# xUhEngwAng/I2V-Adapter-Unofficial

Measured on AMD Instinct MI355X. Metric: denoising steps/sec @ 16fx512x512 SD1.5+I2V-Adapter, higher is better.
Workload: dtype f16

## Files before the change

i2v-adapter-unofficial_amd/_lib.py:

```python
import ctypes as C
import os

_HERE = os.path.dirname(os.path.abspath(__file__))
LIB_PATH = os.environ.get("I2V_LIB_PATH") or os.path.join(_HERE, "libi2v_hip.so")
ABI_VERSION = 11

I2V_EPI_NONE, I2V_EPI_GELU, I2V_EPI_GEGLU = 0, 1, 2
I2V_STORE_ROWMAJOR, I2V_STORE_ROWPERM, I2V_STORE_VT, I2V_STORE_VT_T = 0, 1, 2, 3
I2V_A_PLAIN, I2V_A_CONV3X3 = 0, 1


class HipLibraryError(RuntimeError):
    pass


class GemmParams(C.Structure):
    _fields_ = [
        ("a", C.c_void_p), ("lda", C.c_int64),
        ("a2", C.c_void_p), ("lda2", C.c_int64),
        ("k_split", C.c_int32), ("a_mode", C.c_int32),
        ("w", C.c_void_p), ("ldw", C.c_int64),
        ("bias", C.c_void_p),
        ("residual", C.c_void_p), ("ldr", C.c_int64),
        ("rowvec", C.c_void_p), ("ld_rowvec", C.c_int64), ("rows_per_vec", C.c_int32), ("rowvec_period", C.c_int32),
        ("ln_wsum", C.c_void_p), ("ln_eps", C.c_float),
        ("c", C.c_void_p), ("ldc", C.c_int64),
        ("M", C.c_int32), ("N", C.c_int32), ("K", C.c_int32),
        ("epilogue", C.c_int32), ("store_mode", C.c_int32),
        ("frames", C.c_int32), ("hw", C.c_int32),
        ("vt_len", C.c_int32), ("vt_ld", C.c_int32),
        ("out_scale", C.c_float),
        ("n_img", C.c_int32), ("in_h", C.c_int32), ("in_w", C.c_int32), ("cin", C.c_int32),
        ("out_h", C.c_int32), ("out_w", C.c_int32), ("stride", C.c_int32), ("upsample", C.c_int32),
        ("asym_pad", C.c_int32), ("conv_kblock", C.c_int32),
        ("w_batch_stride", C.c_int64), ("rows_per_w", C.c_int32),
        ("a_perm_frames", C.c_int32), ("a_perm_hw", C.c_int32),
        ("workspace", C.c_void_p), ("workspace_bytes", C.c_int64),
        ("c_is_f32", C.c_int32),
        ("gn_partial", C.c_void_p), ("gn_groups", C.c_int32),
        ("residual_lo", C.c_void_p), ("c_lo", C.c_void_p),
    ]


class AttnParams(C.Structure):
    _fields_ = [
        ("q", C.c_void_p), ("q_row_stride", C.c_int64), ("q_batch_stride", C.c_int64),
        ("k", C.c_void_p), ("k_row_stride", C.c_int64), ("k_batch_stride", C.c_int64),
        ("vt", C.c_void_p), ("vt_row_stride", C.c_int64), ("vt_batch_stride", C.c_int64),
        ("o", C.c_void_p), ("o_row_stride", C.c_int64), ("o_batch_stride", C.c_int64),
        ("batch_q", C.c_int32), ("kv_group", C.c_int32), ("heads", C.c_int32), ("head_dim", C.c_int32),
        ("lq", C.c_int32), ("lk", C.c_int32),
        ("scale", C.c_float), ("accumulate", C.c_int32), ("acc_scale", C.c_float),
        ("lse", C.c_void_p),
    ]


class AttnBwdParams(C.Structure):
    _fields_ = [
        ("q", C.c_void_p), ("q_row_stride", C.c_int64), ("q_batch_stride", C.c_int64),
        ("qt", C.c_void_p), ("qt_row_stride", C.c_int64), ("qt_batch_stride", C.c_int64),
        ("k", C.c_void_p), ("k_row_stride", C.c_int64), ("k_batch_stride", C.c_int64),
        ("kt", C.c_void_p), ("kt_row_stride", C.c_int64), ("kt_batch_stride", C.c_int64),
        ("v", C.c_void_p), ("v_row_stride", C.c_int64), ("v_batch_stride", C.c_int64),
        ("dout", C.c_void_p), ("do_row_stride", C.c_int64), ("do_batch_stride", C.c_int64),
        ("doutt", C.c_void_p), ("dot_row_stride", C.c_int64), ("dot_batch_stride", C.c_int64),
        ("lse", C.c_void_p), ("delta", C.c_void_p),
        ("dq", C.c_void_p), ("dq_row_stride", C.c_int64), ("dq_batch_stride", C.c_int64),
        ("dk", C.c_void_p), ("dk_row_stride", C.c_int64), ("dk_batch_stride", C.c_int64),
        ("dv", C.c_void_p), ("dv_row_stride", C.c_int64), ("dv_batch_stride", C.c_int64),
        ("batch_q", C.c_int32), ("kv_group", C.c_int32), ("heads", C.c_int32), ("head_dim", C.c_int32),
        ("lq", C.c_int32), ("lk", C.c_int32),
        ("scale", C.c_float), ("kv_partitions", C.c_int32), ("dkv_partial", C.c_void_p),
    ]


class TAttnParams(C.Structure):
    _fields_ = [
        ("q", C.c_void_p), ("q_row_stride", C.c_int64),
        ("k", C.c_void_p), ("k_row_stride", C.c_int64),
        ("vt", C.c_void_p), ("vt_ld", C.c_int32),
        ("o", C.c_void_p), ("o_row_stride", C.c_int64),
        ("n_pixels", C.c_int32), ("frames", C.c_int32), ("heads", C.c_int32), ("head_dim", C.c_int32),
        ("scale", C.c_float),
    ]


class MotionAttnParams(C.Structure):
    _fields_ = [
        ("x", C.c_void_p), ("ldx", C.c_int64),
        ("gamma", C.c_void_p),
        ("shift", C.c_void_p), ("ld_shift", C.c_int64),
        ("w_qkv", C.c_void_p),
        ("out", C.c_void_p), ("ldo", C.c_int64),
        ("rows", C.c_int64),
        ("channels", C.c_int32), ("heads", C.c_int32), ("head_dim", C.c_int32), ("frames", C.c_int32),
        ("eps", C.c_float), ("scale", C.c_float),
        ("w_o", C.c_void_p), ("b_o", C.c_void_p),
    ]


class CrossAttnFusedParams(C.Structure):
    _fields_ = [
        ("x", C.c_void_p), ("ldx", C.c_int64),
        ("gamma", C.c_void_p), ("beta", C.c_void_p),
        ("w_q", C.c_void_p),
        ("ctx_frag", C.c_void_p),
        ("out", C.c_void_p), ("ldo", C.c_int64),
        ("rows", C.c_int64), ("rows_per_ctx", C.c_int64),
        ("channels", C.c_int32), ("heads", C.c_int32), ("head_dim", C.c_int32), ("ctx_len", C.c_int32),
        ("eps", C.c_float), ("scale", C.c_float),
        ("ip_frag", C.c_void_p), ("ip_len", C.c_int32), ("ip_scale", C.c_float),
        ("w_o", C.c_void_p), ("b_o", C.c_void_p),
    ]


class FfFusedParams(C.Structure):
    _fields_ = [
        ("x", C.c_void_p), ("ldx", C.c_int64),
        ("gamma", C.c_void_p), ("beta", C.c_void_p),
        ("w1", C.c_void_p), ("b1", C.c_void_p),
        ("w2", C.c_void_p), ("b2", C.c_void_p),
        ("out", C.c_void_p), ("ldo", C.c_int64),
        ("rows", C.c_int64),
        ("channels", C.c_int32), ("inner", C.c_int32),
        ("eps", C.c_float),
        ("w3", C.c_void_p), ("b3", C.c_void_p),
        ("res2", C.c_void_p), ("ld_res2", C.c_int64),
        ("perm_frames", C.c_int32), ("perm_hw", C.c_int32),
        ("res2_lo", C.c_void_p), ("out_lo", C.c_void_p),
    ]


class LnQkvParams(C.Structure):
    _fields_ = [
        ("x", C.c_void_p), ("ldx", C.c_int64),
        ("gamma", C.c_void_p), ("beta", C.c_void_p),
        ("w", C.c_void_p),
        ("qk", C.c_void_p), ("ld_qk", C.c_int64),
        ("vt", C.c_void_p), ("vt_batch_stride", C.c_int64), ("vt_row_stride", C.c_int64),
        ("rows", C.c_int64), ("rows_per_image", C.c_int64),
        ("channels", C.c_int32), ("n_qk", C.c_int32),
        ("eps", C.c_float),
        ("x_image_stride", C.c_int64),
    ]


class UnetConfig(C.Structure):
    _fields_ = [
        ("in_channels", C.c_int32), ("out_channels", C.c_int32),
        ("block_out_channels", C.c_int32 * 4),
        ("layers_per_block", C.c_int32), ("num_attention_heads", C.c_int32),
        ("cross_attention_dim", C.c_int32), ("norm_num_groups", C.c_int32),
        ("motion_max_seq_length", C.c_int32), ("motion_num_attention_heads", C.c_int32),
        ("use_motion_mid_block", C.c_int32), ("ip_num_tokens", C.c_int32),
    ]


class UnetPlan(C.Structure):
    _fields_ = [
        ("batch", C.c_int32), ("frames", C.c_int32), ("height", C.c_int32), ("width", C.c_int32),
        ("ctx_len", C.c_int32), ("has_ip", C.c_int32),
    ]


class GnParams(C.Structure):
    _fields_ = [
        ("x", C.c_void_p), ("c1", C.c_int32),
        ("x2", C.c_void_p), ("c2", C.c_int32),
        ("gamma", C.c_void_p), ("beta", C.c_void_p),
        ("y", C.c_void_p),
        ("n_img", C.c_int32), ("hw", C.c_int32), ("groups", C.c_int32), ("frames_per_stat", C.c_int32),
        ("eps", C.c_float), ("silu", C.c_int32),
        ("out_perm", C.c_int32), ("frames", C.c_int32),
        ("workspace", C.c_void_p),
        ("gpartial_in", C.c_void_p), ("gpartial_rows", C.c_int32),
    ]


class LnParams(C.Structure):
    _fields_ = [
        ("x", C.c_void_p), ("ldx", C.c_int64),
        ("gamma", C.c_void_p), ("beta", C.c_void_p),
        ("pe", C.c_void_p), ("ld_pe", C.c_int64), ("pe_period", C.c_int32),
        ("y", C.c_void_p), ("ldy", C.c_int64),
        ("rows", C.c_int32), ("C", C.c_int32),
        ("eps", C.c_float),
        ("x_rows_per_batch", C.c_int32), ("x_batch_stride", C.c_int64),
    ]


_P = C.c_void_p
SIGNATURES = {
    "i2v_abi_version": (C.c_int, []),
    "i2v_last_error": (C.c_char_p, []),
    "i2v_gemm_f16": (C.c_int, [C.POINTER(GemmParams), _P]),
    "i2v_gemm_ln_supported": (C.c_int, [C.POINTER(GemmParams)]),
    "i2v_gemm_batch_supported": (C.c_int, [C.POINTER(GemmParams)]),
    "i2v_gemm_upconv_fold_supported": (C.c_int, [C.POINTER(GemmParams)]),
    "i2v_gemm_workspace_bytes": (C.c_int64, [C.POINTER(GemmParams)]),
    "i2v_gemm_gn_partial_rows": (C.c_int32, [C.POINTER(GemmParams)]),
    "i2v_attention_f16": (C.c_int, [C.POINTER(AttnParams), _P]),
    "i2v_temporal_attention_f16": (C.c_int, [C.POINTER(TAttnParams), _P]),
    "i2v_motion_attn_supported": (C.c_int32, [C.c_int64, C.c_int32, C.c_int32, C.c_int32, C.c_int32]),
    "i2v_motion_attn_pack_rows": (C.c_int32, [C.c_int32, C.c_int32]),
    "i2v_motion_attn_f16": (C.c_int, [C.POINTER(MotionAttnParams), _P]),
    "i2v_cross_attn_fused_supported": (C.c_int32, [C.c_int64, C.c_int32, C.c_int32, C.c_int32, C.c_int32, C.c_int64]),
    "i2v_cross_attn_fused_pack_rows": (C.c_int32, [C.c_int32, C.c_int32]),
    "i2v_cross_attn_fused_ctx_elems": (C.c_int64, [C.c_int32, C.c_int32, C.c_int32]),
    "i2v_cross_attn_fused_f16": (C.c_int, [C.POINTER(CrossAttnFusedParams), _P]),
    "i2v_ln_qkv_supported": (C.c_int32, [C.c_int64, C.c_int32, C.c_int32, C.c_int64]),
    "i2v_ln_qkv_f16": (C.c_int, [C.POINTER(LnQkvParams), _P]),
    "i2v_ff_fused_supported": (C.c_int32, [C.c_int64, C.c_int32, C.c_int32]),
    "i2v_ff_fused_tail_supported": (C.c_int32, [C.c_int64, C.c_int32, C.c_int32, C.c_int32, C.c_int32]),
    "i2v_ff_fused_f16": (C.c_int, [C.POINTER(FfFusedParams), _P]),
    "i2v_groupnorm_workspace_bytes": (C.c_int64, [C.c_int32, C.c_int32, C.c_int32]),
    "i2v_groupnorm_f16": (C.c_int, [C.POINTER(GnParams), _P]),
    "i2v_groupnorm_fold_f16": (C.c_int, [C.POINTER(GnParams), _P, C.c_int64, _P, C.c_int32, _P, _P, _P]),
    "i2v_layernorm_f16": (C.c_int, [C.POINTER(LnParams), _P]),
    "i2v_softmax_rows_f16": (C.c_int, [_P, C.c_int64, _P, C.c_int64, C.c_int32, C.c_int32, C.c_float, _P]),
    "i2v_nchw_to_tokens": (C.c_int, [_P, C.c_int32, _P, C.c_int32, C.c_int32, C.c_int32, C.c_int32, _P]),
    "i2v_tokens_to_nchw": (C.c_int, [_P, C.c_int32, C.c_int64, _P, C.c_int32, C.c_int32, C.c_int32, C.c_int32, _P]),
    "i2v_timestep_embedding": (C.c_int, [_P, _P, C.c_int32, _P, C.c_int32, C.c_int32, _P]),
    "i2v_silu_f16": (C.c_int, [_P, _P, C.c_int64, _P]),
    "i2v_repeat_rows_f16": (C.c_int, [_P, _P, C.c_int64, C.c_int64, C.c_int32, _P]),
    "i2v_copy3d_f16": (C.c_int, [_P, C.c_int64, C.c_int64, _P, C.c_int64, C.c_int64, C.c_int64, C.c_int64,
                                 C.c_int64, _P]),
    "i2v_pack_ctx_fragments_elems": (C.c_int64, [C.c_int32, C.c_int32, C.c_int32]),
    "i2v_pack_ctx_fragments_f16": (C.c_int, [_P, C.c_int64, _P, C.c_int64, C.c_int64, _P, C.c_int32, C.c_int32, C.c_int32, C.c_int32, _P]),
    "i2v_ddim_prep": (C.c_int, [_P, _P, _P, C.c_int32, C.c_int32, C.c_int32, C.c_int32, C.c_int32, C.c_int32, _P]),
    "i2v_gaussian_sample_f32": (C.c_int, [_P, _P, _P, C.c_int32, C.c_int32, C.c_int32, _P]),
    "i2v_first_frame_prior_f32": (C.c_int, [_P, _P, _P, _P, C.c_int32, C.c_int32, C.c_int32, C.c_int32, C.c_int32,
                                            C.c_float, C.c_float, C.c_float, C.c_float, C.c_float, _P]),
    "i2v_attention_lse_f32": (C.c_int, [C.POINTER(AttnParams), _P, _P]),
    "i2v_attention_bwd_f16": (C.c_int, [C.POINTER(AttnBwdParams), _P]),
    "i2v_transpose_f16": (C.c_int, [_P, C.c_int64, C.c_int64, _P, C.c_int64, C.c_int64, C.c_int32, C.c_int32, C.c_int32, _P]),
    "i2v_rowdot_heads_f32": (C.c_int, [_P, C.c_int64, _P, C.c_int64, _P, C.c_int64, C.c_int32, C.c_int32, C.c_int32, _P]),
    "i2v_layernorm_bwd_f16": (C.c_int, [_P, C.c_int64, _P, C.c_int64, _P, _P, C.c_int64, _P, C.c_int64, C.c_int32, C.c_int32,
                                        C.c_float, _P]),
    "i2v_geglu_bwd_f16": (C.c_int, [_P, C.c_int64, _P, C.c_int64, _P, C.c_int64, C.c_int64, C.c_int32, _P]),
    "i2v_geglu_f16": (C.c_int, [_P, C.c_int64, _P, C.c_int64, C.c_int64, C.c_int32, _P]),
    "i2v_colsum_f32": (C.c_int, [_P, C.c_int64, _P, C.c_int64, C.c_int32, _P]),
    "i2v_colsum_prod_f32": (C.c_int, [_P, C.c_int64, _P, C.c_int64, _P, C.c_int64, C.c_int32, _P]),
    "i2v_colsum_workspace_bytes": (C.c_int64, [C.c_int64, C.c_int32]),
    "i2v_colsum_det_f32": (C.c_int, [_P, C.c_int64, _P, C.c_int64, _P, C.c_int64, C.c_int32, _P, _P]),
    "i2v_masked_mse_grad_f16": (C.c_int, [_P, _P, _P, C.c_int64, C.c_int32, C.c_int32, C.c_int32, C.c_float, _P]),
    "i2v_masked_mse_grad_f32": (C.c_int, [_P, _P, _P, _P, C.c_int64, C.c_int32, C.c_int32, C.c_int32, C.c_float, _P]),
    "i2v_groupnorm_bwd_workspace_bytes": (C.c_int64, [C.c_int32, C.c_int32, C.c_int32]),
    "i2v_groupnorm_bwd_f16": (C.c_int, [C.POINTER(GnParams), _P, _P, _P, _P]),
    "i2v_add_f16": (C.c_int, [_P, _P, _P, C.c_int64, _P]),
    "i2v_permute_rows_f16": (C.c_int, [_P, _P, C.c_int64, C.c_int32, C.c_int32, C.c_int32, C.c_int32, _P]),
    "i2v_zero_insert2x_f16": (C.c_int, [_P, _P, C.c_int64, C.c_int32, C.c_int32, C.c_int32, _P]),
    "i2v_sum_pool2x_f16": (C.c_int, [_P, _P, C.c_int64, C.c_int32, C.c_int32, C.c_int32, _P]),
    "i2v_sumsq_f32": (C.c_int, [_P, C.c_int64, _P, _P]),
    "i2v_adamw_f32": (C.c_int, [_P, _P, _P, _P, C.c_int64, C.c_float, C.c_float, C.c_float, C.c_float, C.c_float, C.c_int32,
                                C.c_float, _P, C.c_float, _P]),
    "i2v_adamw_guarded_f32": (C.c_int, [_P, _P, _P, _P, C.c_int64, C.c_float, C.c_float, C.c_float, C.c_float, C.c_float,
                                        C.c_float, C.c_float, _P, C.c_int32, _P, _P, _P, _P]),
    "i2v_axpby_f32": (C.c_int, [_P, _P, C.c_float, C.c_float, C.c_int64, _P]),
    "i2v_select_row_f16": (C.c_int, [_P, C.c_int64, C.c_int32, _P, _P, C.c_int32, _P]),
    "i2v_ddim_cfg_step": (C.c_int, [_P, _P, C.c_int32, C.c_int64, _P, C.c_int32, _P, C.c_float, C.c_int32, C.c_int32,
                                    C.c_int32, C.c_int32, C.c_int32, _P]),
    "i2v_dpm_cfg_step": (C.c_int, [_P, _P, _P, C.c_int32, C.c_int64, _P, C.c_int32, _P, C.c_float, C.c_int32, C.c_int32,
                                   C.c_int32, C.c_int32, C.c_int32, _P]),
    "i2v_freeu_f16": (C.c_int, [_P, _P, _P, _P, _P, _P, C.c_int32, C.c_int32, C.c_int32, C.c_int32, C.c_int32, C.c_float, C.c_float, _P]),
    "i2v_unet_create": (C.c_int, [C.POINTER(UnetConfig), C.POINTER(_P)]),
    "i2v_unet_destroy": (C.c_int, [_P]),
    "i2v_unet_set_weight": (C.c_int, [_P, C.c_char_p, _P, C.c_int32, C.c_int32, C.POINTER(C.c_int64)]),
    "i2v_unet_get_weight": (C.c_int, [_P, C.c_char_p, C.POINTER(_P), C.POINTER(C.c_int32), C.POINTER(C.c_int32),
                                      C.POINTER(C.c_int64)]),
    "i2v_unet_num_weights": (C.c_int64, [_P]),
    "i2v_unet_plan": (C.c_int, [_P, C.POINTER(UnetPlan)]),
    "i2v_unet_set_plan": (C.c_int, [_P, C.c_char_p, C.c_int64]),
    "i2v_unet_activation_bytes": (C.c_int64, [_P]),
    "i2v_unet_plan_launches": (C.c_int32, [_P]),
    "i2v_unet_plan_num_keys": (C.c_int32, [_P]),
    "i2v_unet_plan_key": (C.c_char_p, [_P, C.c_int32]),
    "i2v_unet_set_workspace": (C.c_int, [_P, _P, C.c_int64]),
    "i2v_unet_forward": (C.c_int, [_P, _P, _P, _P, _P, _P, _P]),
    "i2v_unet_abort_capture": (C.c_int, [_P]),
    "i2v_unet_run": (C.c_int, [_P, C.POINTER(_P), C.c_int32, _P]),
    "i2v_unet_capture_step": (C.c_int, [_P, _P]),
    "i2v_unet_end_capture": (C.c_int, [_P]),
    "i2v_unet_replay_step": (C.c_int, [_P, _P]),
    "i2v_unet_has_step": (C.c_int32, [_P]),
}

_lib = None


def load():
    global _lib
    if _lib is not None:
        return _lib
    if not os.path.exists(LIB_PATH):
        raise HipLibraryError(
            f"{LIB_PATH} not found: the HIP extension is not built.  Run `python __graft_entry__.py build` "
            "(needs hipcc, cross-compiles gfx950 without a GPU).  There is no CPU fallback for this path.")
    try:
        lib = C.CDLL(LIB_PATH)
    except OSError as e:
        raise HipLibraryError(f"cannot load {LIB_PATH}: {e}") from e
    for name, (res, args) in SIGNATURES.items():
        try:
            fn = getattr(lib, name)
        except AttributeError as e:
            raise HipLibraryError(f"{LIB_PATH} does not export `{name}` declared in include/i2v_hip.h") from e
        fn.restype = res
        fn.argtypes = args
    v = lib.i2v_abi_version()
    if v != ABI_VERSION:
        raise HipLibraryError(f"{LIB_PATH} has ABI version {v}, binding expects {ABI_VERSION}")
    _lib = lib
    return lib


def check(status: int, what: str):
    if status != 0:
        msg = load().i2v_last_error()
        raise HipLibraryError(f"{what} failed with status {status}: {msg.decode() if msg else ''}")
```

i2v-adapter-unofficial_amd/blocks.py:

```python
import math
import os
from typing import Optional

import torch
from torch import nn

from . import kernels as K
from . import streams
from ._lib import (I2V_EPI_GEGLU, I2V_EPI_GELU, I2V_EPI_NONE, I2V_STORE_ROWPERM, HipLibraryError)
from .checkpoint import PretrainedMixin

f16 = torch.float16


class HipModule(nn.Module):

    def __init__(self):
        super().__init__()
        self._packed = None
        self._packed_key = None

    def _pack(self):
        return {}

    def __getstate__(self):
        state = self.__dict__.copy()
        state["_packed"], state["_packed_key"] = None, None
        return state

    def packed(self):
        key = tuple((p.data_ptr(), p._version, p.dtype) for p in self.parameters())
        key += tuple((b.data_ptr(), b._version) for b in self.buffers())
        if self._packed is None or key != self._packed_key:
            for p in self.parameters():
                if not p.is_cuda:
                    raise HipLibraryError(
                        f"{type(self).__name__} has parameters on {p.device}: the HIP path has no CPU fallback")
            with torch.no_grad():
                self._packed = self._pack()
            self._packed_key = key
        return self._packed


def w16(t: torch.Tensor) -> torch.Tensor:
    return t.detach().to(f16).contiguous()


class LazyPack(dict):

    def __init__(self, *a, **kw):
        super().__init__(*a, **kw)
        self._lazy = {}

    def lazy(self, name, fn):
        self._lazy[name] = (fn, None)

    def lazy_group(self, names, fn):
        for i, n in enumerate(names):
            self._lazy[n] = (fn, (tuple(names), i))

    def __missing__(self, key):
        if key not in self._lazy:
            raise KeyError(key)
        fn, grp = self._lazy[key]
        with torch.no_grad():
            val = fn()
        if grp is None:
            del self._lazy[key]
            self[key] = val
        else:
            for n, v in zip(grp[0], val):
                self._lazy.pop(n, None)
                dict.__setitem__(self, n, v)
        return dict.__getitem__(self, key)

    def __contains__(self, key):
        return dict.__contains__(self, key) or key in self._lazy

    def get(self, key, default=None):
        return self[key] if key in self else default


def pack_conv3x3(weight: torch.Tensor, cin_pad: Optional[int] = None) -> torch.Tensor:
    co, ci = weight.shape[:2]
    w = weight.detach().permute(0, 2, 3, 1)
    if cin_pad is not None and cin_pad != ci:
        w = torch.nn.functional.pad(w, (0, cin_pad - ci))
        ci = cin_pad
    if K.conv_k_block(ci):
        w = w.reshape(co, 9, ci // 64, 64).permute(0, 2, 1, 3)
    return w.reshape(co, 9 * ci).to(f16).contiguous()


def pack_upconv_fold(weight: torch.Tensor, dtype=f16) -> torch.Tensor:
    co, ci = weight.shape[:2]
    w = weight.detach()
    w = w.double() if w.dtype == torch.float64 else w.float()
    rows = (((0,), (1, 2)), ((0, 1), (2,)))
    phases = []
    for py in range(2):
        for px in range(2):
            taps = []
            for ty in range(2):
                for tx in range(2):
                    acc = None
                    for ky in rows[py][ty]:
                        for kx in rows[px][tx]:
                            acc = w[:, :, ky, kx] if acc is None else acc + w[:, :, ky, kx]
                    taps.append(acc)
            phases.append(torch.stack(taps, dim=1))
    f = torch.stack(phases, dim=0)
    if K.conv_k_block(ci):
        f = f.reshape(4, co, 4, ci // 64, 64).permute(0, 1, 3, 2, 4)
    return f.reshape(4, co, 4 * ci).to(dtype).contiguous()


UPCONV_FOLD = os.environ.get("I2V_UPCONV_FOLD", "1") != "0"


def pack_geglu(weight, bias):
    inner = weight.shape[0] // 2
    w = torch.stack([weight[:inner], weight[inner:]], dim=1).reshape(2 * inner, weight.shape[1])
    b = torch.stack([bias[:inner], bias[inner:]], dim=1).reshape(2 * inner)
    return w16(w), w16(b)


LN_FOLD = os.environ.get("I2V_LN_FOLD", "1") != "0"


def fold_layernorm(weight, bias, gamma, beta):
    wf = (weight.detach().float() * gamma.detach().float()[None, :]).to(f16).contiguous()
    wsum = wf.float().sum(dim=1).contiguous()
    b = weight.detach().float() @ beta.detach().float()
    if bias is not None:
        b = b + bias.detach().float()
    return wf, wsum, b.to(f16).contiguous()


def fold_layernorm_geglu(proj_weight, proj_bias, gamma, beta):
    wf, wsum, b = fold_layernorm(proj_weight, proj_bias, gamma, beta)
    inner = wf.shape[0] // 2
    il = lambda t: torch.stack([t[:inner], t[inner:]], dim=1).reshape((2 * inner,) + tuple(t.shape[1:])).contiguous()
    return il(wf), il(wsum), il(b)


class LnFoldPlan:

    def __init__(self):
        self._cache = {}

    def get(self, key, probe):
        if not LN_FOLD:
            return False
        if key not in self._cache:
            self._cache[key] = bool(probe())
        return self._cache[key]


class ProjectedContext:

    def __init__(self, text, ip):
        self.text, self.ip = text, ip
        self.kv = {}
        self.frag = {}

    @property
    def shape(self):
        return self.text.shape


class ProjectedTemb:

    def __init__(self, all_proj, slices):
        self.all_proj, self.slices = all_proj, slices

    def view_for(self, resnet):
        off, n = self.slices[resnet]
        return self.all_proj[:, off: off + n]

    def first_half(self):
        r = self.all_proj.shape[0]
        return self if r == 1 else ProjectedTemb(self.all_proj[: r // 2], self.slices)


GN_FOLD = os.environ.get("I2V_GN_FOLD", "1") != "0"
GN_FOLD_RATIO = float(os.environ.get("I2V_GN_FOLD_RATIO", "4"))


def gn_proj_in(x, gamma, beta, groups, eps, w, bias, frames=0):
    n, hh, ww, c = x.shape
    hw = hh * ww
    fps = frames if frames > 0 else 1
    s_groups, n_out = n // fps, w.shape[0]
    if GN_FOLD and GN_FOLD_RATIO * s_groups * n_out <= n * hw:
        kw = dict(rows_per_vec=fps * hw, w_rows=fps * hw, a_perm=(frames, hw) if frames > 0 else None)
        if _fold_supported(x, s_groups, n_out, kw):
            w_s, b_s = K.groupnorm_fold(x, gamma, beta, groups, eps, w, bias, frames_per_stat=fps)
            return K.gemm(x.view(-1, c), w_s, None, rowvec=b_s, **kw)
    if frames > 0:
        h = K.groupnorm(x, gamma, beta, groups, eps, frames_per_stat=frames, out_perm=True, frames=frames)
    else:
        h = K.groupnorm(x, gamma, beta, groups, eps).view(-1, c)
    return K.gemm(h, w, bias)


_FOLD_OK = {}


def _fold_supported(x, s_groups, n_out, kw):
    key = (tuple(x.shape), s_groups, n_out, kw["w_rows"], kw["a_perm"])
    ok = _FOLD_OK.get(key)
    if ok is None:
        c = x.shape[3]
        w_s = torch.empty((s_groups, n_out, c), dtype=f16, device=x.device)
        b_s = torch.empty((s_groups, n_out), dtype=f16, device=x.device)
        ok = _FOLD_OK[key] = K.gemm(x.view(-1, c), w_s, None, rowvec=b_s, query_batch_support=True, **kw)
    return ok


def to_tokens(x: torch.Tensor, c_pad: Optional[int] = None) -> torch.Tensor:
    return K.nchw_to_tokens(x, c_pad)


def from_tokens(x: torch.Tensor, dtype) -> torch.Tensor:
    return K.tokens_to_nchw(x, dtype=dtype if dtype in (torch.float32, f16) else f16)


def _as_f16_matrix(t: torch.Tensor) -> torch.Tensor:
    if not t.is_cuda:
        raise HipLibraryError(f"tensor on {t.device}: the HIP path has no CPU fallback")
    return t.to(f16).contiguous()


class Timesteps(nn.Module):

    def __init__(self, num_channels: int, flip_sin_to_cos: bool = True, downscale_freq_shift: float = 0):
        super().__init__()
        if not flip_sin_to_cos or downscale_freq_shift != 0:
            raise NotImplementedError("hot path uses Timesteps(C, flip_sin_to_cos=True, freq_shift=0)")
        self.num_channels = num_channels

    def forward(self, timesteps: torch.Tensor) -> torch.Tensor:
        return K.timestep_embedding(timesteps.to(torch.float32).contiguous(), self.num_channels)


class TimestepEmbedding(HipModule):

    def __init__(self, in_channels: int, time_embed_dim: int, act_fn: str = "silu"):
        super().__init__()
        self.linear_1 = nn.Linear(in_channels, time_embed_dim)
        self.act = nn.SiLU()
        self.linear_2 = nn.Linear(time_embed_dim, time_embed_dim)

    def _pack(self):
        return dict(w1=w16(self.linear_1.weight), b1=w16(self.linear_1.bias), w2=w16(self.linear_2.weight),
                    b2=w16(self.linear_2.bias))

    def forward(self, sample, condition=None):
        p = self.packed()
        h = K.silu(K.gemm(_as_f16_matrix(sample), p["w1"], p["b1"]))
        return K.gemm(h, p["w2"], p["b2"])


_PRECISE_STREAM = os.environ.get("I2V_STREAM_PRECISE", "0") != "0"


def precise_stream() -> bool:
    return _PRECISE_STREAM


def set_precise_stream(on: bool) -> bool:
    global _PRECISE_STREAM
    prev, _PRECISE_STREAM = _PRECISE_STREAM, bool(on)
    return prev


GN_FROM_CONV = os.environ.get("I2V_GN_FROM_CONV", "1") != "0"


class ResnetBlock2D(HipModule):

    def __init__(self, in_channels, out_channels=None, temb_channels=512, eps=1e-6, groups=32,
                 output_scale_factor=1.0, **_unused):
        super().__init__()
        out_channels = in_channels if out_channels is None else out_channels
        self.in_channels, self.out_channels = in_channels, out_channels
        self.output_scale_factor = output_scale_factor
        self.groups, self.eps = groups, eps
        self.norm1 = nn.GroupNorm(groups, in_channels, eps=eps, affine=True)
        self.conv1 = nn.Conv2d(in_channels, out_channels, 3, stride=1, padding=1)
        self.time_emb_proj = nn.Linear(temb_channels, out_channels) if temb_channels is not None else None
        self.norm2 = nn.GroupNorm(groups, out_channels, eps=eps, affine=True)
        self.conv2 = nn.Conv2d(out_channels, out_channels, 3, stride=1, padding=1)
        self.nonlinearity = nn.SiLU()
        self.conv_shortcut = (nn.Conv2d(in_channels, out_channels, 1, stride=1, padding=0)
                              if in_channels != out_channels else None)

    def _pack(self):
        p = dict(g1=w16(self.norm1.weight), b1=w16(self.norm1.bias), w1=pack_conv3x3(self.conv1.weight),
                 cb1=w16(self.conv1.bias), g2=w16(self.norm2.weight), b2=w16(self.norm2.bias),
                 w2=pack_conv3x3(self.conv2.weight), cb2=w16(self.conv2.bias))
        if self.time_emb_proj is not None:
            p["wt"], p["bt"] = w16(self.time_emb_proj.weight), w16(self.time_emb_proj.bias)
        if self.conv_shortcut is not None:
            p["ws"] = w16(self.conv_shortcut.weight.reshape(self.out_channels, self.in_channels))
            p["bs"] = w16(self.conv_shortcut.bias)
        return p

    def _fwd(self, x, temb_act, x2=None):
        p = self.packed()
        n, hh, ww, c1 = x.shape
        cin = c1 + (x2.shape[3] if x2 is not None else 0)
        if cin != self.in_channels:
            raise ValueError(f"ResnetBlock2D expects {self.in_channels} input channels, got {cin}")
        if self.conv_shortcut is None and x2 is not None:
            raise ValueError("concat input needs a conv_shortcut")
        s = x
        with streams.fork(self.conv_shortcut is not None and n * hh * ww <= streams.MAX_ROWS, x.device) as fk:
            if self.conv_shortcut is not None:
                with fk.side():
                    a2 = None if x2 is None else x2.view(-1, x2.shape[3])
                    s = K.sview(K.gemm(x.view(-1, c1), p["ws"], p["bs"], a2=a2, precise=precise_stream()), n, hh, ww, self.out_channels)
            h = K.groupnorm(x, p["g1"], p["b1"], self.groups, self.eps, x2=x2, silu=True)
            rowvec, rpv = None, 0
            if self.time_emb_proj is not None and temb_act is not None:
                rowvec = (temb_act.view_for(self) if isinstance(temb_act, ProjectedTemb)
                          else K.gemm(temb_act, p["wt"], p["bt"]))
                rpv = (n // rowvec.shape[0]) * hh * ww
            if GN_FROM_CONV:
                h, st = K.conv3x3(h, p["w1"], p["cb1"], rowvec=rowvec, rows_per_vec=rpv, gn_stats_groups=self.groups)
            else:
                h, st = K.conv3x3(h, p["w1"], p["cb1"], rowvec=rowvec, rows_per_vec=rpv), None
            h = K.groupnorm(h, p["g2"], p["b2"], self.groups, self.eps, silu=True, stats=st)
        return K.conv3x3(h, p["w2"], p["cb2"], residual=s, out_scale=1.0 / self.output_scale_factor, precise=precise_stream())

    def forward(self, input_tensor, temb, scale: float = 1.0):
        x = to_tokens(input_tensor)
        ta = K.silu(_as_f16_matrix(temb)) if temb is not None else None
        return from_tokens(self._fwd(x, ta), input_tensor.dtype)


class Downsample2D(HipModule):

    def __init__(self, channels, use_conv=True, out_channels=None, padding=1, name="conv"):
        super().__init__()
        if not use_conv or padding not in (0, 1):
            raise NotImplementedError("Downsample2D(use_conv=True, padding in {0, 1}) only")
        out_channels = out_channels or channels
        self.padding = padding
        self.conv = nn.Conv2d(channels, out_channels, 3, stride=2, padding=padding)

    def _pack(self):
        return dict(w=pack_conv3x3(self.conv.weight), b=w16(self.conv.bias))

    def _fwd(self, x):
        p = self.packed()
        return K.conv3x3(x, p["w"], p["b"], stride=2, asym_pad=self.padding == 0, precise=precise_stream())

    def forward(self, hidden_states, scale: float = 1.0):
        return from_tokens(self._fwd(to_tokens(hidden_states)), hidden_states.dtype)


class Upsample2D(HipModule):

    def __init__(self, channels, use_conv=True, out_channels=None):
        super().__init__()
        if not use_conv:
            raise NotImplementedError("hot path uses Upsample2D(use_conv=True)")
        out_channels = out_channels or channels
        self.conv = nn.Conv2d(channels, out_channels, 3, padding=1)

    def _pack(self):
        p = LazyPack(w=pack_conv3x3(self.conv.weight), b=w16(self.conv.bias))
        p.lazy("w_fold", lambda: pack_upconv_fold(self.conv.weight))
        return p

    def _fwd(self, x, output_size=None):
        p = self.packed()
        size = None if output_size is None else tuple(int(v) for v in output_size)
        if (UPCONV_FOLD and size in (None, (2 * x.shape[1], 2 * x.shape[2]))
                and K.upconv_fold_supported(x.shape, self.conv.out_channels)):
            return K.conv3x3(x, p["w"], p["b"], upsample=True, w_folded=p["w_fold"])
        return K.conv3x3(x, p["w"], p["b"], upsample=True, output_size=size)

    def forward(self, hidden_states, output_size=None, scale: float = 1.0):
        return from_tokens(self._fwd(to_tokens(hidden_states), output_size), hidden_states.dtype)


class Attention(HipModule):

    def __init__(self, query_dim, cross_attention_dim=None, heads=8, dim_head=64, bias=False, out_bias=True,
                 dropout=0.0, upcast_attention=False):
        super().__init__()
        if bias:
            raise NotImplementedError("attention_bias=True is not on the hot path")
        self.inner_dim = dim_head * heads
        self.heads, self.dim_head = heads, dim_head
        self.query_dim = query_dim
        self.cross_attention_dim = cross_attention_dim if cross_attention_dim is not None else query_dim
        self.scale = dim_head ** -0.5
        self.to_q = nn.Linear(query_dim, self.inner_dim, bias=False)
        self.to_k = nn.Linear(self.cross_attention_dim, self.inner_dim, bias=False)
        self.to_v = nn.Linear(self.cross_attention_dim, self.inner_dim, bias=False)
        self.to_out = nn.ModuleList([nn.Linear(self.inner_dim, query_dim, bias=out_bias), nn.Dropout(dropout)])
        self.ip_num_tokens, self.ip_scale = 0, 1.0
        self.to_k_ip = None
        self.to_v_ip = None

    def install_ip_adapter(self, to_k_ip_weight, to_v_ip_weight, num_tokens=4, scale=1.0):
        dev, dt = self.to_q.weight.device, self.to_q.weight.dtype
        self.to_k_ip = nn.Linear(self.cross_attention_dim, self.inner_dim, bias=False).to(device=dev, dtype=dt)
        self.to_v_ip = nn.Linear(self.cross_attention_dim, self.inner_dim, bias=False).to(device=dev, dtype=dt)
        with torch.no_grad():
            self.to_k_ip.weight.copy_(to_k_ip_weight)
            self.to_v_ip.weight.copy_(to_v_ip_weight)
        self.ip_num_tokens, self.ip_scale = num_tokens, scale

    def _pack(self):
        ob = self.to_out[0].bias
        p = dict(wq=w16(self.to_q.weight), wk=w16(self.to_k.weight), wv=w16(self.to_v.weight),
                 wo=w16(self.to_out[0].weight), bo=None if ob is None else w16(ob))
        if self.to_k_ip is not None:
            p["wk_ip"], p["wv_ip"] = w16(self.to_k_ip.weight), w16(self.to_v_ip.weight)
        return p

    def project_kv(self, ctx_text, ctx_ip, out=None):
        p = self.packed()
        bc, lt, dc = ctx_text.shape
        o = out if out is not None else (None, None, None, None)
        k = K.gemm(ctx_text.view(-1, dc), p["wk"], out=o[0])
        vt = K.project_vt(ctx_text.view(-1, dc), p["wv"], lt, out=o[1])
        kip = vtip = None
        if ctx_ip is not None and self.ip_num_tokens:
            kip = K.gemm(ctx_ip.view(-1, dc), p["wk_ip"], out=o[2])
            vtip = K.project_vt(ctx_ip.view(-1, dc), p["wv_ip"], ctx_ip.shape[1], out=o[3])
        return k, vt, kip, vtip

    def context_kv(self, ctx_text, ctx_ip):
        if isinstance(ctx_text, ProjectedContext):
            k, vt, kip, vtip = ctx_text.kv[self]
            lt = ctx_text.text.shape[1]
            li = ctx_text.ip.shape[1] if ctx_text.ip is not None else 0
        else:
            k, vt, kip, vtip = self.project_kv(ctx_text, ctx_ip)
            lt = ctx_text.shape[1]
            li = ctx_ip.shape[1] if ctx_ip is not None else 0
        return k, vt, kip, vtip, lt, li

    def context_fragments(self, ctx_text, kv):
        k, vt, kip, vtip, lt, li = kv
        use_ip = kip is not None and bool(self.ip_num_tokens)
        if not isinstance(ctx_text, ProjectedContext):
            return K.pack_ctx_fragments(k, vt, self.heads, lt), (K.pack_ctx_fragments(kip, vtip, self.heads, li) if use_ip else None)
        hit = ctx_text.frag.get(self)
        if hit is None:
            hit = ctx_text.frag[self] = (K.pack_ctx_fragments(k, vt, self.heads, lt),
                                         K.pack_ctx_fragments(kip, vtip, self.heads, li) if use_ip else None)
        return hit

    def refresh_context_fragments(self, pc):
        hit = pc.frag.get(self)
        if hit is not None:
            k, vt, kip, vtip, lt, li = self.context_kv(pc, None)
            K.pack_ctx_fragments(k, vt, self.heads, lt, out=hit[0])
            if hit[1] is not None:
                K.pack_ctx_fragments(kip, vtip, self.heads, li, out=hit[1])

    def _cross(self, q, ctx_text, ctx_ip, batch_q, lq, kv_group, kv=None):
        k, vt, kip, vtip, lt, li = kv if kv is not None else self.context_kv(ctx_text, ctx_ip)
        o = K.attention(q, k, vt, batch_q=batch_q, lq=lq, lk=lt, heads=self.heads, head_dim=self.dim_head,
                        kv_group=kv_group, scale=self.scale)
        if kip is not None and self.ip_num_tokens:
            K.attention(q, kip, vtip, batch_q=batch_q, lq=lq, lk=li, heads=self.heads, head_dim=self.dim_head,
                        kv_group=kv_group, scale=self.scale, out=o, accumulate=True, acc_scale=self.ip_scale)
        return o

    def forward(self, hidden_states, encoder_hidden_states=None, attention_mask=None):
        if attention_mask is not None:
            raise NotImplementedError("attention masks are never passed on the hot path (SURVEY 8b)")
        p = self.packed()
        x = _as_f16_matrix(hidden_states)
        b, l, c = x.shape
        q = K.gemm(x.view(-1, c), p["wq"])
        ctx = x if encoder_hidden_states is None else _as_f16_matrix(encoder_hidden_states)
        ctx_ip = None
        if self.ip_num_tokens and encoder_hidden_states is not None:
# ... 656 lines not shown
```

i2v-adapter-unofficial_amd/csrc/gemm.hip:

```cpp
#include <cstdlib>

#include "gemm_common.h"

namespace {

constexpr int BK = 64;

template <int BM, int BN>
struct Smem {
  f16 a[2][BM * BK];
  f16 w[2][BN * BK];
};

__device__ __forceinline__ int swz(int row, int chunk) { return row * 128 + ((chunk ^ ((row >> 1) & 7)) << 4); }

struct ConvRow {
  int pix_base;
  int oy, ox;
  bool valid;
};

template <int BM, int BN, int AMODE>
__global__ __launch_bounds__(256) void gemm_kernel(const i2v_gemm_params p, const int tiles_n, const int vec4) {
  constexpr int WM = BM / 2, WN = BN / 2, MI = WM / 16, NI = WN / 16;
// ... 185 lines not shown
          for (int r = 0; r < 4; ++r) v[r] += (float)b4[r];
        }
        if (rv) {
          const f16x4 t4 = *reinterpret_cast<const f16x4*>(rv + n);
#pragma unroll
          for (int r = 0; r < 4; ++r) v[r] += (float)t4[r];
        }
        if (rs) {
          const f16x4 r4 = *reinterpret_cast<const f16x4*>(rs + n);
#pragma unroll
          for (int r = 0; r < 4; ++r) v[r] += (float)r4[r];
          if (rl) {
            const f16x4 l4 = *reinterpret_cast<const f16x4*>(rl + n);
#pragma unroll
            for (int r = 0; r < 4; ++r) v[r] += (float)l4[r];
          }
        }
      } else {
#pragma unroll
        for (int r = 0; r < 4; ++r) {
          if (n + r < N) {
            if (bias) v[r] += (float)bias[n + r];
            if (rv) v[r] += (float)rv[n + r];
            if (rs) v[r] += (float)rs[n + r];
            if (rl) v[r] += (float)rl[n + r];
          }
        }
      }
      if (p.epilogue == I2V_EPI_GEGLU) {
        const float o0 = v[0] * gelu_erf(v[1]) * oscale;
        const float o1 = v[2] * gelu_erf(v[3]) * oscale;
        f16* dst = C + m_out * p.ldc + (n >> 1);
        if (vec4) {
          f16x2 o = {(f16)o0, (f16)o1};
          *reinterpret_cast<f16x2*>(dst) = o;
        } else {
          if (n + 1 < N) dst[0] = (f16)o0;
          if (n + 3 < N) dst[1] = (f16)o1;
        }
        continue;
      }
#pragma unroll
      for (int r = 0; r < 4; ++r) {
        if (p.epilogue == I2V_EPI_GELU) v[r] = gelu_erf(v[r]);
        v[r] *= oscale;
      }
      if (p.store_mode == I2V_STORE_VT_T) {
        const int bt = m / p.vt_len, kk = m - bt * p.vt_len;
#pragma unroll
        for (int r = 0; r < 4; ++r)
          if (n + r < N) C[((int64_t)bt * N + (n + r)) * p.vt_ld + kk] = (f16)v[r];
      } else if (p.store_mode == I2V_STORE_VT) {
        if (vec4) {
          const int bt = n / p.vt_len, kk = n - bt * p.vt_len;
          f16x4 o = {(f16)v[0], (f16)v[1], (f16)v[2], (f16)v[3]};
          *reinterpret_cast<f16x4*>(C + ((int64_t)bt * M + m) * p.vt_ld + kk) = o;
        } else {
#pragma unroll
          for (int r = 0; r < 4; ++r) {
            if (n + r < N) {
              const int bt = (n + r) / p.vt_len, kk = (n + r) - bt * p.vt_len;
              C[((int64_t)bt * M + m) * p.vt_ld + kk] = (f16)v[r];
            }
          }
        }
      } else if (p.c_is_f32) {
        float* dst = reinterpret_cast<float*>(p.c) + m_out * p.ldc + n;
        if (vec4) {
          *reinterpret_cast<f32x4*>(dst) = f32x4{v[0], v[1], v[2], v[3]};
        } else {
#pragma unroll
          for (int r = 0; r < 4; ++r)
            if (n + r < N) dst[r] = v[r];
        }
      } else {
        f16* dst = C + m_out * p.ldc + n;
        if (vec4) {
          f16x4 o = {(f16)v[0], (f16)v[1], (f16)v[2], (f16)v[3]};
          *reinterpret_cast<f16x4*>(dst) = o;
          if (cl) *reinterpret_cast<f16x4*>(cl + n) = f16x4{lo_half(v[0], o[0]), lo_half(v[1], o[1]), lo_half(v[2], o[2]), lo_half(v[3], o[3])};
        } else {
#pragma unroll
          for (int r = 0; r < 4; ++r)
            if (n + r < N) {
              dst[r] = (f16)v[r];
              if (cl) cl[n + r] = lo_half(v[r], (f16)v[r]);
            }
        }
      }
    }
  }
}

struct TileCfg {
  int bm, bn, blocks_per_cu;
  float eff;
};

template <int BM, int BN>
int launch(const i2v_gemm_params& p, int vec4, hipStream_t s) {
  const int tiles_m = (int)i2v_cdiv(p.M, BM), tiles_n = (int)i2v_cdiv(p.N, BN);
  const dim3 grid(tiles_m * tiles_n), block(256);
  if (p.a_mode == I2V_A_CONV3X3)
    hipLaunchKernelGGL((gemm_kernel<BM, BN, I2V_A_CONV3X3>), grid, block, 0, s, p, tiles_n, vec4);
  else
    hipLaunchKernelGGL((gemm_kernel<BM, BN, I2V_A_PLAIN>), grid, block, 0, s, p, tiles_n, vec4);
  return i2v_check_launch("i2v_gemm_f16");
}

inline bool aligned_to(const void* p, uintptr_t a) { return (reinterpret_cast<uintptr_t>(p) % a) == 0; }

int vector_epilogue_ok(const i2v_gemm_params& p) {
  int vec4 = (p.N % 4 == 0) ? 1 : 0;
  if (p.bias && !aligned_to(p.bias, 8)) vec4 = 0;
  if (p.residual && (!aligned_to(p.residual, 8) || p.ldr % 4 != 0)) vec4 = 0;
  if ((p.residual_lo && !aligned_to(p.residual_lo, 8)) || (p.c_lo && !aligned_to(p.c_lo, 8))) vec4 = 0;
  if (p.rowvec && (!aligned_to(p.rowvec, 8) || p.ld_rowvec % 4 != 0)) vec4 = 0;
  if (p.store_mode == I2V_STORE_VT) {
    if (p.vt_len % 4 != 0 || p.vt_ld % 4 != 0 || !aligned_to(p.c, 8)) vec4 = 0;
  } else if (p.store_mode == I2V_STORE_VT_T) {
    vec4 = (p.vt_len % 4 == 0 && p.vt_ld % 4 == 0 && aligned_to(p.c, 8) && p.M % 4 == 0) ? 1 : 0;
  } else if (p.epilogue == I2V_EPI_GEGLU) {
    if (p.ldc % 2 != 0 || !aligned_to(p.c, 4)) vec4 = 0;
  } else if (p.c_is_f32) {
    if (p.ldc % 4 != 0 || !aligned_to(p.c, 16)) vec4 = 0;
  } else {
    if (p.ldc % 4 != 0 || !aligned_to(p.c, 8)) vec4 = 0;
  }
  return vec4;
}

}

extern "C" int64_t i2v_gemm_workspace_bytes(const i2v_gemm_params* pp) {
  if (pp == nullptr || pp->M <= 0 || pp->N <= 0 || pp->K <= 0) return 0;
  return i2v_gemm_big_plan(*pp, vector_epilogue_ok(*pp)).workspace_bytes;
}

extern "C" int i2v_gemm_ln_supported(const i2v_gemm_params* pp) {
  if (pp == nullptr || pp->M <= 0 || pp->N <= 0 || pp->K <= 0) return 0;
  return i2v_gemm_big_plan(*pp, vector_epilogue_ok(*pp)).ln_fold ? 1 : 0;
}

extern "C" int i2v_gemm_batch_supported(const i2v_gemm_params* pp) {
  if (pp == nullptr || pp->M <= 0 || pp->N <= 0 || pp->K <= 0) return 0;
  return i2v_gemm_big_plan(*pp, vector_epilogue_ok(*pp)).form == GemmBigForm::Tile ? 1 : 0;
}

extern "C" int i2v_gemm_upconv_fold_supported(const i2v_gemm_params* pp) {
  if (pp == nullptr || pp->M <= 0 || pp->N <= 0 || pp->K <= 0 || pp->a_mode != I2V_A_CONV3X3 || pp->upsample != 2) return 0;
  return i2v_gemm_big_plan(*pp, vector_epilogue_ok(*pp)).form == GemmBigForm::Tile ? 1 : 0;
}

extern "C" int32_t i2v_gemm_gn_partial_rows(const i2v_gemm_params* pp) {
  if (pp == nullptr) return 0;
  return i2v_gemm_big_plan(*pp, vector_epilogue_ok(*pp)).gn_rows;
}

extern "C" int i2v_gemm_f16(const i2v_gemm_params* pp, i2v_stream_t stream) {
  I2V_CHECK_ARG(pp != nullptr, "i2v_gemm_f16: null params");
  const i2v_gemm_params& p = *pp;
  I2V_CHECK_ARG(p.a && p.w && p.c, "i2v_gemm_f16: null a/w/c pointer");
  I2V_CHECK_ARG(p.M > 0 && p.N > 0 && p.K > 0, "i2v_gemm_f16: M, N, K must be positive (got %d, %d, %d)", p.M, p.N,
                p.K);
  I2V_CHECK_ARG(p.K % 8 == 0, "i2v_gemm_f16: K (%d) must be a multiple of 8", p.K);
  I2V_CHECK_ARG(p.ldw % 8 == 0 && p.ldw >= p.K, "i2v_gemm_f16: ldw (%lld) must be >= K and a multiple of 8",
                (long long)p.ldw);
  I2V_CHECK_ARG(aligned_to(p.a, 16) && aligned_to(p.w, 16), "i2v_gemm_f16: a / w must be 16-byte aligned");
  I2V_CHECK_ARG(p.lda % 8 == 0, "i2v_gemm_f16: lda (%lld) must be a multiple of 8", (long long)p.lda);
  if (p.a_mode == I2V_A_CONV3X3) {
    I2V_CHECK_ARG(p.a2 == nullptr, "i2v_gemm_f16: conv mode takes a single source");
    I2V_CHECK_ARG(p.upsample >= 0 && p.upsample <= 2, "i2v_gemm_f16: upsample must be 0, 1 or 2 (got %d)", p.upsample);
    I2V_CHECK_ARG(p.cin > 0 && p.cin % 8 == 0 && p.K == (p.upsample == 2 ? 4 : 9) * p.cin,
                  "i2v_gemm_f16: conv needs cin %% 8 == 0, K == 9 cin (4 cin with the up-sampling folded into the weights)");
    I2V_CHECK_ARG(p.stride == 1 || p.stride == 2, "i2v_gemm_f16: conv stride must be 1 or 2");
    I2V_CHECK_ARG(!(p.upsample && p.stride != 1), "i2v_gemm_f16: upsample conv must have stride 1");
    I2V_CHECK_ARG(!p.asym_pad || (p.stride == 2 && !p.upsample), "i2v_gemm_f16: asym_pad needs stride 2, no upsample");
    I2V_CHECK_ARG(p.conv_kblock == 0 || (p.conv_kblock == 64 && p.cin % 64 == 0),
                  "i2v_gemm_f16: conv_kblock must be 0 or 64 (with cin %% 64 == 0), got %d for cin %d", p.conv_kblock, p.cin);
    const int padsum = p.asym_pad ? 1 : 2;
    const int eh = p.upsample ? 2 * p.in_h : (p.in_h + padsum - 3) / p.stride + 1;
    const int ew = p.upsample ? 2 * p.in_w : (p.in_w + padsum - 3) / p.stride + 1;
    I2V_CHECK_ARG((p.out_h == eh || (p.upsample == 1 && p.out_h == eh - 1)) && (p.out_w == ew || (p.upsample == 1 && p.out_w == ew - 1)),
                  "i2v_gemm_f16: conv output size mismatch (%d x %d vs %d x %d)", p.out_h, p.out_w, eh, ew);
    I2V_CHECK_ARG((int64_t)p.n_img * p.out_h * p.out_w == p.M, "i2v_gemm_f16: conv M != n_img*out_h*out_w");
    I2V_CHECK_ARG(p.lda >= p.cin, "i2v_gemm_f16: conv pixel stride lda < cin");
    I2V_CHECK_ARG((int64_t)p.n_img * p.in_h * p.in_w < (1ll << 31), "i2v_gemm_f16: conv image too large");
  } else {
    I2V_CHECK_ARG(p.a_mode == I2V_A_PLAIN, "i2v_gemm_f16: bad a_mode %d", p.a_mode);
    if (p.a2) {
      I2V_CHECK_ARG(p.k_split > 0 && p.k_split < p.K && p.k_split % 8 == 0 && p.lda2 % 8 == 0 && aligned_to(p.a2, 16),
                    "i2v_gemm_f16: bad dual-source split (k_split %d, K %d)", p.k_split, p.K);
      I2V_CHECK_ARG(p.lda >= p.k_split && p.lda2 >= p.K - p.k_split, "i2v_gemm_f16: dual-source ld too small");
    } else {
      I2V_CHECK_ARG(p.lda >= p.K, "i2v_gemm_f16: lda (%lld) < K (%d)", (long long)p.lda, p.K);
    }
  }
  I2V_CHECK_ARG(p.epilogue >= I2V_EPI_NONE && p.epilogue <= I2V_EPI_GEGLU, "i2v_gemm_f16: bad epilogue");
  I2V_CHECK_ARG(p.store_mode >= I2V_STORE_ROWMAJOR && p.store_mode <= I2V_STORE_VT_T, "i2v_gemm_f16: bad store_mode");
  if (p.epilogue == I2V_EPI_GEGLU)
    I2V_CHECK_ARG(p.N % 2 == 0 && p.store_mode != I2V_STORE_VT && p.store_mode != I2V_STORE_VT_T,
                  "i2v_gemm_f16: GEGLU needs even N, non-VT store");
  if (p.store_mode == I2V_STORE_VT_T) {
    I2V_CHECK_ARG(p.vt_len > 0 && p.vt_ld >= p.vt_len && p.M % p.vt_len == 0,
                  "i2v_gemm_f16: VT_T store needs M %% vt_len == 0 and vt_ld >= vt_len");
    I2V_CHECK_ARG(p.residual == nullptr && (p.rowvec == nullptr || (p.rowvec_period > 0 && p.ln_wsum)),
                  "i2v_gemm_f16: VT_T store takes no residual, and a rowvec only as the transposed positional table of a "
                  "LayerNorm-folded projection");
  }
  if (p.c_is_f32)
    I2V_CHECK_ARG(p.c_is_f32 == 1 && p.epilogue != I2V_EPI_GEGLU && p.store_mode == I2V_STORE_ROWMAJOR && p.ln_wsum == nullptr &&
                      p.rows_per_w == 0 && p.a_perm_frames == 0 && p.N <= 64 && aligned_to(p.c, 4),
                  "i2v_gemm_f16: an fp32 result (c_is_f32) is a row-major store of a narrow (N <= 64), plain problem");
  if (p.residual_lo || p.c_lo) {
    I2V_CHECK_ARG(p.residual_lo == nullptr || p.residual != nullptr, "i2v_gemm_f16: residual_lo needs residual");
    I2V_CHECK_ARG(p.epilogue == I2V_EPI_NONE && (p.store_mode == I2V_STORE_ROWMAJOR || p.store_mode == I2V_STORE_ROWPERM) && !p.c_is_f32 &&
                      p.ln_wsum == nullptr && p.gn_partial == nullptr,
                  "i2v_gemm_f16: the precise residual stream (residual_lo / c_lo) takes plain row-major / row-permuted fp16 stores only");
  }
  if (p.rowvec) I2V_CHECK_ARG(p.rows_per_vec > 0 || p.rowvec_period > 0, "i2v_gemm_f16: rows_per_vec must be positive");
  if (p.store_mode == I2V_STORE_ROWPERM) {
    I2V_CHECK_ARG(p.frames > 0 && p.hw > 0 && p.M % (p.frames * p.hw) == 0,
                  "i2v_gemm_f16: ROWPERM needs M %% (frames*hw) == 0");
    I2V_CHECK_ARG(p.rowvec == nullptr, "i2v_gemm_f16: ROWPERM does not take rowvec");
  }
  if (p.store_mode == I2V_STORE_VT) {
    I2V_CHECK_ARG(p.vt_len > 0 && p.vt_ld >= p.vt_len && p.N % p.vt_len == 0,
                  "i2v_gemm_f16: VT store needs N %% vt_len == 0 and vt_ld >= vt_len");
    I2V_CHECK_ARG(p.residual == nullptr && p.rowvec == nullptr, "i2v_gemm_f16: VT store takes no residual/rowvec");
  }

  int vec4 = vector_epilogue_ok(p);
  const GemmBigPlan big_plan = i2v_gemm_big_plan(p, vec4);
  if (p.rowvec && p.rowvec_period > 0)
    I2V_CHECK_ARG(p.store_mode != I2V_STORE_ROWPERM && p.store_mode != I2V_STORE_VT &&
                      (p.rowvec_period & (p.rowvec_period - 1)) == 0,
                  "i2v_gemm_f16: a periodic rowvec (positional table) needs a power-of-two period (the epilogue masks the "
                  "row index: an integer modulo there cost the 256-row kernels 40 %%) and a row-major / VT_T store");
  if (p.ln_wsum) {
    I2V_CHECK_ARG(aligned_to(p.ln_wsum, 16) && p.ln_eps > 0.f, "i2v_gemm_f16: ln_wsum must be 16-byte aligned, ln_eps > 0");
    if (!big_plan.ln_fold)
      I2V_FAIL(I2V_ERR_INVALID_ARG, "i2v_gemm_f16: LayerNorm-folded GEMM is not implemented for this problem "
               "(M %d N %d K %d, epilogue %d, store %d): ask i2v_gemm_ln_supported() first", p.M, p.N, p.K, p.epilogue,
               p.store_mode);
  }

  if (p.gn_partial) {
    I2V_CHECK_ARG(aligned_to(p.gn_partial, 8), "i2v_gemm_f16: gn_partial must be 8-byte aligned");
    if (!big_plan.gn_rows)
      I2V_FAIL(I2V_ERR_INVALID_ARG, "i2v_gemm_f16: GroupNorm partials (gn_partial) are not implemented for this problem (M %d N %d K %d, "
               "groups %d): ask i2v_gemm_gn_partial_rows() first", p.M, p.N, p.K, p.gn_groups);
  }
  if (p.a_mode == I2V_A_CONV3X3 && p.upsample == 2 && big_plan.form != GemmBigForm::Tile)
    I2V_FAIL(I2V_ERR_INVALID_ARG, "i2v_gemm_f16: the folded up-sampling convolution (upsample = 2) is not implemented for this problem "
             "(M %d N %d cin %d, %d x %d -> %d x %d, rows_per_w %d): ask i2v_gemm_upconv_fold_supported() first", p.M, p.N, p.cin,
             p.in_h, p.in_w, p.out_h, p.out_w, p.rows_per_w);
  if (p.rows_per_w > 0 || p.a_perm_frames > 0) {
    I2V_CHECK_ARG(p.rows_per_w >= 0 && p.a_perm_frames >= 0 && p.w_batch_stride >= 0, "i2v_gemm_f16: negative batch / permutation field");
    if (big_plan.form != GemmBigForm::Tile)
      I2V_FAIL(I2V_ERR_INVALID_ARG, "i2v_gemm_f16: per-batch weights / the permuted A gather are not implemented for this "
               "problem (M %d N %d K %d, rows_per_w %d, a_perm %d x %d): they need the 8-wave kernel with full row tiles",
               p.M, p.N, p.K, p.rows_per_w, p.a_perm_frames, p.a_perm_hw);
  }
#ifdef I2V_VARIANTS
  {
    const int ws = i2v_gemm_ws_try(p, reinterpret_cast<hipStream_t>(stream));
    if (ws != 0) return ws < 0 ? ws : I2V_OK;
  }
#endif
  {
    const int thin = i2v_conv_thin_try(p, reinterpret_cast<hipStream_t>(stream));
    if (thin != 0) return thin < 0 ? thin : I2V_OK;
  }
  {
    const int big = i2v_gemm_big_launch(p, vec4, big_plan, reinterpret_cast<hipStream_t>(stream));
    if (big != 0) return big < 0 ? big : I2V_OK;
  }
  if (p.store_mode == I2V_STORE_VT_T) vec4 = 0;
  const bool conv = p.a_mode == I2V_A_CONV3X3;
  const bool long_k = p.K >= 2048;
  const TileCfg cfgs[4] = {{128, 128, 2, long_k ? 1.15f : 1.00f},
                           {128, 64, 3, conv ? 1.00f : 1.30f},
                           {64, 128, 3, conv ? 1.25f : 1.25f},
                           {64, 64, 5, 1.10f}};
  int best = 0;
  double best_t = 1e300;
  for (int i = 0; i < 4; ++i) {
    const double tiles = (double)i2v_cdiv(p.M, cfgs[i].bm) * (double)i2v_cdiv(p.N, cfgs[i].bn);
    const double slots = 256.0 * cfgs[i].blocks_per_cu;
    const double rounds = tiles <= slots ? 1.0 : tiles / slots;
    const double conc = tiles < slots ? tiles : slots;
    const double per_cu = (conc / 256.0 < 1.0) ? 1.0 : conc / 256.0;
    const double t = rounds * per_cu * cfgs[i].bm * cfgs[i].bn / cfgs[i].eff;
    if (t < best_t) {
      best_t = t;
      best = i;
    }
  }
  static const int tile_env = getenv("I2V_GEMM_TILE") ? atoi(getenv("I2V_GEMM_TILE")) : -1;
  if (tile_env >= 0 && tile_env < 4) best = tile_env;
  hipStream_t s = reinterpret_cast<hipStream_t>(stream);
  switch (best) {
    case 0: return launch<128, 128>(p, vec4, s);
    case 1: return launch<128, 64>(p, vec4, s);
    case 2: return launch<64, 128>(p, vec4, s);
    default: return launch<64, 64>(p, vec4, s);
  }
}
```

i2v-adapter-unofficial_amd/csrc/gemm_big.hip:

```cpp
#include <algorithm>
#include <cstdlib>
#include <utility>

#include "gemm_common.h"

namespace {

constexpr int BIG_BN = 320;

__device__ __forceinline__ void bdma16(__amdgpu_buffer_rsrc_t rsrc, char* lds_wave_base, unsigned voff, int soff) {
  __builtin_amdgcn_raw_ptr_buffer_load_lds(rsrc, (__attribute__((address_space(3))) void*)lds_wave_base, 16, voff, soff, 0,
                                           0);
}

__device__ __forceinline__ int fast_div(int m, int d, float inv_d) {
  int q = (int)((float)m * inv_d);
  const int r = m - q * d;
  q += (r >= d) ? 1 : 0;
  q -= (r < 0) ? 1 : 0;
  return q;
}

__device__ __forceinline__ float xor_sum(float x, int partner_addr) {
  return x + __builtin_bit_cast(float, __builtin_amdgcn_ds_bpermute(partner_addr, __builtin_bit_cast(int, x)));
}
__device__ __forceinline__ float uniform_f(float x) {
  return __builtin_bit_cast(float, __builtin_amdgcn_readfirstlane(__builtin_bit_cast(int, x)));
}

#ifndef I2V_CONV_COLMAJOR
#define I2V_CONV_COLMAJOR 1
#endif
#ifndef I2V_GEMM_PANEL
#define I2V_GEMM_PANEL 8
#endif

template <int N>
__device__ __forceinline__ void wait_vmcnt() {
  asm volatile("s_waitcnt vmcnt(%0)" ::"n"(N) : "memory");
}

template <int N, class F, int... Is>
__device__ __forceinline__ void static_for_impl(F&& f, std::integer_sequence<int, Is...>) {
  (f(std::integral_constant<int, Is>{}), ...);
}
template <int N, class F>
__device__ __forceinline__ void static_for(F&& f) {
  static_for_impl<N>(f, std::make_integer_sequence<int, N>{});
}

template <int BK>
__device__ __forceinline__ int big_lds_addr(int row, int kchunk) {
  const int u = BK == 64 ? row : row >> 1;
  const int c8 = BK == 64 ? kchunk : ((row & 1) << 2) + kchunk;
  return u * 128 + ((c8 ^ ((u >> 1) & 7)) << 4);
}

template <int BM, int BK, int NS, int AMODE, int EPI, int STORE, bool SPLIT = false, bool STAGGER = true, bool LNF = false,
          bool FAST = false, int BNT = 320, int NW = 8, bool GNS = false, bool HILO = false, bool UPF = false>
__global__ __launch_bounds__(NW * 64, NW == 4 ? 2 : 1) void gemm_big_kernel(const i2v_gemm_params p, const int tiles_n,
                                                                            const int kps, const int ntiles) {
  static_assert(NS == 2 || (NS <= 4 && !FAST && !SPLIT && NW == 8),
                "the cross-tile prefetch of the persistent tile loop, the LayerNorm fold and split-K are written for two stages");
  static_assert(NW == 8 || (NW == 4 && !STAGGER && !SPLIT), "4-wave workgroups: one M-wave, no stagger partner, no split-K");
  static_assert(!UPF || (AMODE == I2V_A_CONV3X3 && EPI == I2V_EPI_NONE && STORE == I2V_STORE_ROWMAJOR && !SPLIT && !LNF && !FAST &&
                         !GNS && !HILO && NW == 8),
                "the folded up-sampling convolution is an un-split conv with the plain row-contiguous store");
  constexpr int BN = BNT;
  constexpr int WNC = BN / 4;
  constexpr int WM = BM / (NW / 4), MI = WM / 16, NI = WNC / 16;
  static_assert(BN % 64 == 0 && (BN == 320 || (!LNF && !SPLIT)), "the LayerNorm fold and split-K are written for BN = 320");
  constexpr int AG = BM * BK / (512 * NW);
  constexpr int WGT = BN * BK * 2 / 1024;
  constexpr int WG = (WGT + NW - 1) / NW;
  static_assert(AG >= 1 && (BM * BK) % (512 * NW) == 0, "the A tile must be whole 1 KiB groups per wave");
  constexpr int STAGE = (BM + BN) * BK * 2;
  constexpr int KSTEPS = BK / 32;
  __shared__ __attribute__((aligned(16))) char smem[NS * STAGE + 1024 + (LNF ? 2048 + 512 + 2 * 1280 : 0)];
  float2* const lds_st = reinterpret_cast<float2*>(smem + NS * STAGE + 1024);
  float* const lds_ws2 = reinterpret_cast<float*>(smem + NS * STAGE + 1024 + 2048 + 512);

#if defined(I2V_PROBE) && I2V_PROBE == 5
  long long stamp[6], cstamp[6];
#define I2V_STAMP(i) stamp[i] = __builtin_amdgcn_s_memrealtime(); cstamp[i] = __builtin_amdgcn_s_memtime()
#else
#define I2V_STAMP(i)
#endif
  const int tid = threadIdx.x, lane = tid & 63;
  const int wave = __builtin_amdgcn_readfirstlane(tid >> 6);
  const int wm = wave >> 2, wn = wave & 3;
  const int g = lane >> 4, l15 = lane & 15;
  const int M = p.M, N = p.N, K = p.K;

  const f16* __restrict__ A = reinterpret_cast<const f16*>(p.a);
  const f16* __restrict__ A2 = reinterpret_cast<const f16*>(p.a2);
  const f16* __restrict__ W = reinterpret_cast<const f16*>(p.w);
  const int ksp = (A2 != nullptr) ? p.k_split : K;

  constexpr unsigned OOB = 0x80000000u;
  constexpr int RSTEP = (BK == 64 ? 8 : 16) * NW;
  const int lr = lane >> 3, lc = lane & 7;
  const int u0 = 8 * wave + lr;
  const int c8 = lc ^ ((u0 >> 1) & 7);
  const int r0 = BK == 64 ? u0 : 2 * u0 + (c8 >> 2);
  const int lane_k = (BK == 64 ? c8 : (c8 & 3)) * 8;
  const int n_wbatch = p.rows_per_w > 0 ? M / p.rows_per_w : 1;
  const auto rs_w = __builtin_amdgcn_make_buffer_rsrc(
      const_cast<f16*>(W), 0, (int)(((int64_t)(n_wbatch - 1) * p.w_batch_stride + (int64_t)(N - 1) * p.ldw + K) * 2), 0x00020000);
  const int64_t a_extent = AMODE == I2V_A_CONV3X3 ? ((int64_t)p.n_img * p.in_h * p.in_w - 1) * p.lda + p.cin
                                                  : (int64_t)(M - 1) * p.lda + ksp;
  const auto rs_a = __builtin_amdgcn_make_buffer_rsrc(const_cast<f16*>(A), 0, (int)(a_extent * 2), 0x00020000);
  const auto rs_a2 = __builtin_amdgcn_make_buffer_rsrc(
      const_cast<f16*>(A2 ? A2 : A), 0, A2 ? (int)(((int64_t)(M - 1) * p.lda2 + (K - ksp)) * 2) : 0, 0x00020000);
  const int pf = p.a_perm_frames;
  const int pf_shift = pf > 0 ? 31 - __builtin_clz(pf) : 0;
  const unsigned a_lane = pf > 0 ? (unsigned)((((r0 & (pf - 1)) * p.a_perm_hw + (r0 >> pf_shift)) * (int)p.lda + lane_k) * 2)
                                 : (unsigned)((r0 * (int)p.lda + lane_k) * 2);
  const unsigned w_lane = (unsigned)((r0 * (int)p.ldw + lane_k) * 2);
  auto conv_rows = [&](int tm0, int (&cp)[AG], int (&cy)[AG], int (&cx)[AG]) {
    if constexpr (UPF) {
      const int mq = M >> 2, ph = tm0 / mq, ihw = p.in_h * p.in_w;
#pragma unroll
      for (int i = 0; i < AG; ++i) {
        const int mm = tm0 - ph * mq + r0 + RSTEP * i;
        const int img = mm / ihw, rem = mm - img * ihw, sy = rem / p.in_w;
        cp[i] = img * ihw;
        cy[i] = sy - 1 + (ph >> 1);
        cx[i] = rem - sy * p.in_w - 1 + (ph & 1);
      }
      return;
    }
#pragma unroll
    for (int i = 0; i < AG; ++i) {
      const int m = tm0 + r0 + RSTEP * i;
      const bool ok = m < M;
      const int ohw = p.out_h * p.out_w;
      const int mm = ok ? m : 0;
      const int img = mm / ohw, rem = mm - img * ohw;
      cp[i] = img * p.in_h * p.in_w;
      cy[i] = ok ? rem / p.out_w : -4;
      cx[i] = rem - (rem / p.out_w) * p.out_w;
    }
  };

  auto issue_at = [&](int kt, int stage, int tm0, int tn0, const int (&cp)[AG], const int (&cy)[AG], const int (&cx)[AG]) {
    char* sa = smem + stage * STAGE;
    char* sw = sa + BM * BK * 2;
    const int kb = kt * BK;
    if (AMODE == I2V_A_CONV3X3) {
      int tap, ci;
      if (UPF && p.conv_kblock) {
        tap = kt & 3;
        ci = (kt >> 2) * BK;
      } else if (p.conv_kblock) {
        tap = kt % 9;
        ci = (kt / 9) * BK;
      } else {
        tap = kb / p.cin;
        ci = kb - tap * p.cin;
      }
      const int dy = UPF ? tap >> 1 : tap / 3, dx = UPF ? tap & 1 : tap - dy * 3;
#pragma unroll
      for (int i = 0; i < AG; ++i) {
        int iy, ix;
        bool ok;
        if (UPF) {
          iy = cy[i] + dy;
          ix = cx[i] + dx;
          ok = (iy >= 0) && (ix >= 0) && (iy < p.in_h) && (ix < p.in_w);
        } else if (p.upsample) {
          const int uy = cy[i] - 1 + dy, ux = cx[i] - 1 + dx;
          ok = (uy >= 0) && (ux >= 0) && (uy < p.out_h) && (ux < p.out_w);
          iy = uy >> 1;
          ix = ux >> 1;
        } else {
          iy = cy[i] * p.stride - (p.asym_pad ? 0 : 1) + dy;
          ix = cx[i] * p.stride - (p.asym_pad ? 0 : 1) + dx;
          ok = (iy >= 0) && (ix >= 0) && (iy < p.in_h) && (ix < p.in_w);
        }
        const unsigned voff = ok ? (unsigned)(((cp[i] + iy * p.in_w + ix) * (int)p.lda + ci + lane_k) * 2) : OOB;
        bdma16(rs_a, sa + (wave + NW * i) * 1024, voff, 0);
      }
    } else if (FAST || (kb < ksp && tm0 + BM <= M)) {
      int arow0 = tm0, astep = RSTEP;
      if (pf > 0) {
        const int per = pf * p.a_perm_hw;
        const int tb = tm0 / per, tp = (tm0 - tb * per) >> pf_shift;
        arow0 = tb * per + tp;
        astep = RSTEP >> pf_shift;
      }
#pragma unroll
      for (int i = 0; i < AG; ++i) {
        int soff = ((arow0 + astep * i) * (int)p.lda + kb) * 2;
        asm volatile("" : "+s"(soff));
        bdma16(rs_a, sa + (wave + NW * i) * 1024, a_lane, soff);
      }
    } else {
      int ol = lane;
      asm volatile("" : "+v"(ol));
      const int ou0 = 8 * wave + (ol >> 3);
      const int oc8 = (ol & 7) ^ ((ou0 >> 1) & 7);
      const int orow = BK == 64 ? ou0 : 2 * ou0 + (oc8 >> 2);
      const int ok8 = (BK == 64 ? oc8 : (oc8 & 3)) * 8;
      const bool first = kb < ksp;
#pragma unroll
      for (int i = 0; i < AG; ++i) {
        const int m = tm0 + orow + RSTEP * i;
        const unsigned voff = m < M ? (unsigned)((m * (int)(first ? p.lda : p.lda2) + ok8) * 2) : OOB;
        if (first)
          bdma16(rs_a, sa + (wave + NW * i) * 1024, voff, kb * 2);
        else
          bdma16(rs_a2, sa + (wave + NW * i) * 1024, voff, (kb - ksp) * 2);
      }
    }
    const int wb_off = p.rows_per_w > 0 ? (int)((tm0 / p.rows_per_w) * p.w_batch_stride * 2) : 0;
#pragma unroll
    for (int i = 0; i < WG; ++i) {
      const bool in_tile = (WGT % NW == 0) || (wave + NW * i < WGT);
      bdma16(rs_w, in_tile ? sw + (wave + NW * i) * 1024 : smem + NS * STAGE, in_tile ? w_lane : OOB,
             ((tn0 + RSTEP * i) * (int)p.ldw + kb) * 2 + wb_off);
    }
  };

  const int tiles_m_all = ntiles / tiles_n;
  auto tile_coords = [&](int id, int& tm, int& tn) {
    if (I2V_CONV_COLMAJOR && AMODE == I2V_A_CONV3X3) {
      tn = id / tiles_m_all;
      tm = id - tn * tiles_m_all;
    } else if (I2V_GEMM_PANEL > 0 && tiles_n > I2V_GEMM_PANEL && tiles_n % I2V_GEMM_PANEL == 0) {
      const int per_panel = tiles_m_all * I2V_GEMM_PANEL;
      const int panel = id / per_panel, r = id - panel * per_panel;
      tm = r / I2V_GEMM_PANEL;
      tn = panel * I2V_GEMM_PANEL + (r - tm * I2V_GEMM_PANEL);
    } else {
      tm = id / tiles_n;
      tn = id - tm * tiles_n;
    }
  };
  const int nkt_all = (K + BK - 1) / BK;
  const int kt0 = SPLIT ? (int)blockIdx.y * kps : 0;
  const int nkt = SPLIT ? min(nkt_all, kt0 + kps) : nkt_all;
  static_assert(!FAST || (!SPLIT && AMODE == I2V_A_PLAIN && NW == 8), "FAST is a plain, un-split, 8-wave GEMM");
  constexpr bool PERSIST = FAST;
  int sbase = 0;
  bool have_first = false;
  int ws_buf = 0;
  for (int round0 = 0; round0 < ntiles; round0 += (int)gridDim.x) {
  const int in_round = min((int)gridDim.x, ntiles - round0);
  if ((int)blockIdx.x >= in_round) break;
  const int tile = round0 + xcd_remap(blockIdx.x, in_round);
  int tile_m, tile_n;
  tile_coords(tile, tile_m, tile_n);
  const int m0 = tile_m * BM, n0 = tile_n * BN;
  const int next0 = round0 + (int)gridDim.x;
  const bool has_next = PERSIST && next0 < ntiles && (int)blockIdx.x < min((int)gridDim.x, ntiles - next0);
#if defined(I2V_PROBE) && I2V_PROBE == 5
  I2V_STAMP(0);
#endif
  int c_pix[AG], c_oy[AG], c_ox[AG];
  if (AMODE == I2V_A_CONV3X3) {
    conv_rows(m0, c_pix, c_oy, c_ox);
  } else {
#pragma unroll
    for (int i = 0; i < AG; ++i) c_pix[i] = c_oy[i] = c_ox[i] = 0;
  }
  auto issue = [&](int kt, int stage) { issue_at(kt, stage, m0, n0, c_pix, c_oy, c_ox); };
  auto issue_next_first = [&](int stage) {
    const int nt = next0 + xcd_remap(blockIdx.x, min((int)gridDim.x, ntiles - next0));
    int ntm, ntn;
    tile_coords(nt, ntm, ntn);
    issue_at(0, stage, ntm * BM, ntn * BN, c_pix, c_oy, c_ox);
  };

  f32x4 acc[NI][MI];
#pragma unroll
  for (int i = 0; i < NI; ++i)
#pragma unroll
    for (int j = 0; j < MI; ++j) acc[i][j] = f32x4{0.f, 0.f, 0.f, 0.f};

  float* const lds_ws = lds_ws2 + ws_buf * BN;
  if (!have_first) {
#pragma unroll
    for (int st = 0; st < NS - 1; ++st)
      if (kt0 + st < nkt) issue(kt0 + st, (sbase + st) % NS);
  }
  if (LNF) {
    const float* lnws_g = reinterpret_cast<const float*>(p.ln_wsum);
    if (NW == 8) {
      if (tid < BN) {
        const float ln_col = lnws_g[n0 + tid];
        wait_vmcnt<0>();
        lds_ws[tid] = ln_col;
      }
    } else {
      const float c0 = lnws_g[n0 + tid];
      const float c1 = tid < BN - 256 ? lnws_g[n0 + 256 + tid] : 0.f;
      wait_vmcnt<0>();
      lds_ws[tid] = c0;
      if (tid < BN - 256) lds_ws[256 + tid] = c1;
    }
    ws_buf ^= 1;
  }
// ... 412 lines not shown
        }
      });
    });
    I2V_STAMP(3);
    static_for<MI>([&](auto jc) {
      constexpr int j = decltype(jc)::value;
      if constexpr (j + RES_AHEAD < MI && EPI != I2V_EPI_GEGLU && !UPF) {
        fetch_rows(std::integral_constant<int, j + RES_AHEAD>{});
      }
      static_for<NI>([&](auto ic) {
        constexpr int i = decltype(ic)::value;
        if (EPI == I2V_EPI_GEGLU)
          *reinterpret_cast<float2*>(stg + l15 * LDS_LD + i * 8 + 2 * g) = float2{acc[i][j][0], acc[i][j][1]};
        else
          *reinterpret_cast<f32x4*>(stg + l15 * LDS_LD + i * 16 + 4 * g) = acc[i][j];
      });
#pragma unroll
      for (int q = 0; q < QN; ++q) {
        int m, m_out, n;
        const bool ok = task(j, q, m, m_out, n);
        const int t = lane + 64 * q;
        const int row = (t / TPR) & 15, c = t - (t / TPR) * TPR;
        const f32x4 lo = *reinterpret_cast<const f32x4*>(stg + row * LDS_LD + c * 8);
        const f32x4 hi = *reinterpret_cast<const f32x4*>(stg + row * LDS_LD + c * 8 + 4);
        float v[8] = {lo[0], lo[1], lo[2], lo[3], hi[0], hi[1], hi[2], hi[3]};
        if (EPI != I2V_EPI_GEGLU) {
          if (!UPF && has_add) {
#pragma unroll
            for (int e = 0; e < 8; ++e) v[e] += (float)xpre[j][q][e];
            if constexpr (HILO) {
#pragma unroll
              for (int e = 0; e < 8; ++e) v[e] += (float)xlo[j][q][e];
            }
          }
#pragma unroll
          for (int e = 0; e < 8; ++e) v[e] *= oscale;
        }
        f16x8 o;
#pragma unroll
        for (int e = 0; e < 8; ++e) o[e] = (f16)v[e];
        const unsigned off = ok ? (unsigned)((m_out * (int)p.ldc + n) * 2) : EOOB;
        __builtin_amdgcn_raw_buffer_store_b128(__builtin_bit_cast(u32x4, o), rs_c, off, 0, 0);
        if constexpr (HILO) {
          f16x8 ol;
#pragma unroll
          for (int e = 0; e < 8; ++e) ol[e] = (f16)(v[e] - (float)o[e]);
          __builtin_amdgcn_raw_buffer_store_b128(__builtin_bit_cast(u32x4, ol), rs_cl, off, 0, 0);
        }
      }
    });
#if defined(I2V_PROBE) && I2V_PROBE == 5
    I2V_STAMP(4);
    asm volatile("s_waitcnt vmcnt(0)" ::: "memory");
    I2V_STAMP(5);
    if (tid == 0) {
      long long* dst = reinterpret_cast<long long*>(C + (int64_t)m0 * p.ldc + out_col0);
      for (int q = 0; q < 6; ++q) dst[q] = stamp[q];
      for (int q = 0; q < 6; ++q) dst[6 + q] = cstamp[q];
    }
#endif
    return;
  }
  static_for<MI>([&](auto jc) {
    constexpr int j = decltype(jc)::value;
    const int m = m0 + wm * WM + j * 16 + l15;
    if (m < M) {
      int64_t m_out = m;
      if (STORE == I2V_STORE_ROWPERM) {
        const int per = p.hw * p.frames;
        const int b = m / per, rem = m - b * per;
        const int pix = rem / p.frames, f = rem - pix * p.frames;
        m_out = (int64_t)(b * p.frames + f) * p.hw + pix;
      }
      const f16* rv = rowvec ? rowvec + (int64_t)(p.rowvec_period > 0 ? (m & (p.rowvec_period - 1)) : fast_div(m, p.rows_per_vec, inv_rpv)) * p.ld_rowvec
                             : nullptr;
      const f16* rs = resid ? resid + m_out * p.ldr : nullptr;
      static_for<NI>([&](auto ic) {
        constexpr int i = decltype(ic)::value;
        const int n = ncol0 + i * 16;
        float v[4];
#pragma unroll
        for (int r = 0; r < 4; ++r) v[r] = acc[i][j][r] + (float)b4[i][r];
        if (rv) {
          const f16x4 t4 = *reinterpret_cast<const f16x4*>(rv + n);
#pragma unroll
          for (int r = 0; r < 4; ++r) v[r] += (float)t4[r];
        }
        if (rs) {
          const f16x4 r4 = *reinterpret_cast<const f16x4*>(rs + n);
#pragma unroll
          for (int r = 0; r < 4; ++r) v[r] += (float)r4[r];
        }
        if (EPI == I2V_EPI_GEGLU) {
          const f16x2 o2 = {(f16)(v[0] * gelu_erf(v[1]) * oscale), (f16)(v[2] * gelu_erf(v[3]) * oscale)};
          *reinterpret_cast<f16x2*>(C + m_out * p.ldc + (n >> 1)) = o2;
        } else {
          const f16x4 o4 = {(f16)(v[0] * oscale), (f16)(v[1] * oscale), (f16)(v[2] * oscale), (f16)(v[3] * oscale)};
          if (STORE == I2V_STORE_VT) {
            const int bt = n / p.vt_len, kk = n - bt * p.vt_len;
            *reinterpret_cast<f16x4*>(C + ((int64_t)bt * M + m) * p.vt_ld + kk) = o4;
          } else {
            *reinterpret_cast<f16x4*>(C + m_out * p.ldc + n) = o4;
          }
        }
      });
    }
  });
  };
  int e_lane = lane;
  asm volatile("" : "+v"(e_lane));
  epilogue(e_lane, e_lane >> 4, e_lane & 15, wave * 64 + e_lane);
  if (!PERSIST) break;
  }
}

__global__ __launch_bounds__(256) void splitk_reduce_kernel(const i2v_gemm_params p, const int splits, const int vec4) {
  const int64_t groups = (int64_t)p.M * (p.N / 4);
  const float* __restrict__ ws = reinterpret_cast<const float*>(p.workspace);
  const int64_t slab = (int64_t)p.M * p.N;
  for (int64_t i = (int64_t)blockIdx.x * 256 + threadIdx.x; i < groups; i += (int64_t)gridDim.x * 256) {
    const int m = (int)(i / (p.N / 4)), n = (int)(i - (int64_t)m * (p.N / 4)) * 4;
    f32x4 s4 = *reinterpret_cast<const f32x4*>(ws + (int64_t)m * p.N + n);
    for (int sidx = 1; sidx < splits; ++sidx) s4 += *reinterpret_cast<const f32x4*>(ws + sidx * slab + (int64_t)m * p.N + n);
    float v[4] = {s4[0], s4[1], s4[2], s4[3]};
    const GemmRow row = gemm_make_row(p, m);
    gemm_store4(p, vec4, row, n, v);
  }
}


struct GemmBigSwitches {
  int big;
  int splitk;
  int split256;
  int deep;
  int persist;
  int four_wave;
};
const GemmBigSwitches& switches() {
  static const GemmBigSwitches sw = [] {
    auto env = [](const char* name, int unset) { return getenv(name) ? atoi(getenv(name)) : unset; };
    return GemmBigSwitches{env("I2V_GEMM_BIG", -1),    env("I2V_GEMM_SPLITK", 1),  env("I2V_GEMM_SPLIT256", 1),
                           env("I2V_GEMM_DEEP", 2),    env("I2V_GEMM_PERSIST", 0), env("I2V_GEMM_4W", 0)};
  }();
  return sw;
}
constexpr int BIG_MIN_K = 128;
constexpr int SPLIT256_MIN_TILES = 16;
constexpr int DEEP_MIN_KT = 10, DEEP_MAX_KT = 63;
constexpr bool BIG_VAE_TILES = true;

bool upconv_fold(const i2v_gemm_params& p) { return p.a_mode == I2V_A_CONV3X3 && p.upsample == 2; }

struct SplitPlan {
  int splits = 0, kps = 0;
};
SplitPlan even_splits(int nkt, int splits) {
  SplitPlan sp;
  sp.kps = (int)i2v_cdiv(nkt, splits);
  sp.splits = (int)i2v_cdiv(nkt, sp.kps);
  return sp.splits < 2 ? SplitPlan{} : sp;
}

SplitPlan splitk_plan(const i2v_gemm_params& p, int vec4) {
  if (upconv_fold(p)) return {};
  if (p.N % BIG_BN != 0 || !vec4 || p.epilogue != I2V_EPI_NONE || p.store_mode != I2V_STORE_ROWMAJOR) return {};
  const int nkt = (p.K + 63) / 64;
  const int64_t t128 = i2v_cdiv(p.M, 128) * (p.N / BIG_BN);
  if (nkt < 40 || t128 > 128) return {};
  int splits = (int)(256 / t128);
  const int cap = (p.a_mode == I2V_A_PLAIN && nkt >= 256) ? 64 : 8;
  if (splits > cap) splits = cap;
  if (splits > nkt / 8) splits = nkt / 8;
  if (splits < 2) return {};
  return even_splits(nkt, splits);
}

SplitPlan splitk256_plan(const i2v_gemm_params& p, int vec4) {
  const int on = switches().split256;
  if (!on) return {};
  const int nkt = (p.K + 63) / 64;
  const int64_t t256 = (int64_t)(p.M / 256) * (p.N / BIG_BN);
  if (on == 1 && p.a_mode == I2V_A_CONV3X3 && nkt < 90) return {};
  if (on == 1 && p.a_mode != I2V_A_CONV3X3 && t256 > 32) return {};
  if (p.N % BIG_BN != 0 || !vec4 || p.epilogue != I2V_EPI_NONE || p.store_mode != I2V_STORE_ROWMAJOR || p.M % 256 != 0) return {};
  if (p.a2 != nullptr || p.rows_per_w > 0 || p.a_perm_frames > 0 || p.ln_wsum != nullptr) return {};
  if (nkt < 64 || t256 < SPLIT256_MIN_TILES || t256 > 128) return {};
  int splits = (int)(256 / t256);
  if (splits > 8) splits = 8;
  if (splits > nkt / 8) splits = nkt / 8;
  return even_splits(nkt, splits);
}

int deep_cols(const i2v_gemm_params& p, int vec4) {
  if (!switches().deep || !vec4) return 0;
  if (p.a_mode != I2V_A_PLAIN || p.epilogue != I2V_EPI_NONE || p.store_mode == I2V_STORE_VT_T || p.ln_wsum != nullptr) return 0;
  if (p.rows_per_w > 0 || p.a_perm_frames > 0 || p.c_is_f32) return 0;
  if (p.N % 128 != 0 || (p.K + 63) / 64 < DEEP_MIN_KT) return 0;
  const int64_t tm = i2v_cdiv(p.M, 128);
  if (tm * (p.N / 128) <= 256) return 128;
  if (p.N % 256 == 0 && tm * (p.N / 256) <= 256) return 256;
  return 0;
}

bool a16(const void* q) { return (reinterpret_cast<uintptr_t>(q) & 15) == 0; }
bool lo_stream(const i2v_gemm_params& p) { return p.residual_lo != nullptr || p.c_lo != nullptr; }
bool workspace_holds(const i2v_gemm_params& p, int splits) {
  return p.workspace && p.workspace_bytes >= (int64_t)splits * p.M * p.N * (int64_t)sizeof(float) && a16(p.workspace);
}

void plan_form(const i2v_gemm_params& p, int vec4, GemmBigPlan& plan) {
  using Form = GemmBigForm;
  const GemmBigSwitches& sw = switches();
  const bool conv = p.a_mode == I2V_A_CONV3X3;
  auto set = [&plan](Form form, int rows, int cols, int stages, SplitPlan sp = {}) {
    plan.form = form, plan.rows = rows, plan.cols = cols, plan.stages = stages, plan.splits = sp.splits, plan.kps = sp.kps;
  };
  if (sw.big == 0) return;
  if (p.c_is_f32) return;
  const int dcols = deep_cols(p, vec4);
  int cols = 0;
  if (p.N % BIG_BN == 0) {
    cols = BIG_BN;
  } else if (p.a_mode == I2V_A_PLAIN) {
    if (!dcols) return;
  } else if (BIG_VAE_TILES && conv && p.epilogue == I2V_EPI_NONE && p.store_mode == I2V_STORE_ROWMAJOR && !lo_stream(p)) {
    cols = p.N % 256 == 0 ? 256 : p.N % 128 == 0 ? 128 : 0;
    if (!cols) return;
  } else {
    return;
  }
  const bool deep_only = cols == 0;
  if (p.K % 64 != 0 || (p.a2 != nullptr && p.k_split % 64 != 0)) return;
  if ((int64_t)p.N * p.ldw >= (1ll << 30)) return;
  if (conv) {
    if (p.cin % 64 != 0 || (int64_t)p.n_img * p.in_h * p.in_w * p.lda >= (1ll << 30)) return;
    if (p.conv_kblock != 0 && p.conv_kblock != 64) return;
  } else if ((int64_t)p.M * p.lda >= (1ll << 30) || (int64_t)p.M * p.lda2 >= (1ll << 30)) {
    return;
  }
  if (!vec4 || p.epilogue == I2V_EPI_GELU) return;
  if (conv && (p.epilogue != I2V_EPI_NONE || p.store_mode != I2V_STORE_ROWMAJOR)) return;
  if (p.epilogue == I2V_EPI_GEGLU && p.store_mode != I2V_STORE_ROWMAJOR) return;
  if (p.store_mode == I2V_STORE_ROWMAJOR || p.store_mode == I2V_STORE_ROWPERM) {
    if (p.ldc % 8 != 0 || !a16(p.c)) return;
    if (p.residual && (p.ldr % 8 != 0 || !a16(p.residual))) return;
    if (!a16(p.residual_lo) || !a16(p.c_lo)) return;
    if (p.rowvec && (p.ld_rowvec % 8 != 0 || !a16(p.rowvec))) return;
  }
  if (p.rowvec && p.M >= (1 << 24)) return;
  if (p.residual && p.rowvec && p.epilogue != I2V_EPI_GEGLU) return;
  const int64_t rv_rows = p.rowvec_period > 0 ? p.rowvec_period : (p.M - 1) / (p.rows_per_vec > 0 ? p.rows_per_vec : 1) + 1;
  if ((int64_t)p.M * p.ldc >= (1ll << 30) || (p.residual && (int64_t)p.M * p.ldr >= (1ll << 30)) ||
      (p.rowvec && rv_rows * p.ld_rowvec >= (1ll << 30)))
    return;
  const bool fold = upconv_fold(p);
  if (fold) {
    if (p.K != 4 * p.cin || p.stride != 1 || p.out_h != 2 * p.in_h || p.out_w != 2 * p.in_w) return;
    if (p.M % 4 != 0 || p.rows_per_w != p.M / 4 || p.rows_per_w % 256 != 0 || p.a_perm_frames > 0 || p.M >= (1 << 24)) return;
    if (p.w_batch_stride < (int64_t)p.N * p.ldw || 4 * p.w_batch_stride >= (1ll << 30)) return;
    if (p.residual || p.rowvec || lo_stream(p) || p.gn_partial || p.ln_wsum) return;
  } else if (p.rows_per_w > 0 || p.a_perm_frames > 0) {
    if (p.a_mode != I2V_A_PLAIN || p.a2 != nullptr || p.M % 256 != 0) return;
    if (p.rows_per_w > 0 && (p.rows_per_w % 256 != 0 || p.M % p.rows_per_w != 0 ||
                             (int64_t)(p.M / p.rows_per_w) * p.w_batch_stride >= (1ll << 30)))
      return;
    if (p.a_perm_frames > 0) {
      const int f = p.a_perm_frames;
      if ((f & (f - 1)) != 0 || f > 64 || p.a_perm_hw <= 0 || p.a_perm_hw % (64 / f) != 0 ||
          ((int64_t)f * p.a_perm_hw) % 256 != 0 || p.M % (f * p.a_perm_hw) != 0)
        return;
    }
  }
  if (sw.big == 256 || sw.big == 128) {
    if (!deep_only) set(Form::Tile, sw.big, cols, 2);
    return;
  }
  if (!conv && p.K < BIG_MIN_K) return;
  const SplitPlan sp256 = splitk256_plan(p, vec4);
  if (sp256.splits && workspace_holds(p, sp256.splits)) return set(Form::SplitK, 256, BIG_BN, 2, sp256);
  const int64_t tn = deep_only ? i2v_cdiv(p.N, BIG_BN) : p.N / cols;
  const int64_t t256 = i2v_cdiv(p.M, 256) * tn, t128 = i2v_cdiv(p.M, 128) * tn;
  const double e256 = (double)t256 / (double)(i2v_cdiv(t256, 256) * 256);
  const double e128 = 0.82 * (double)t128 / (double)(i2v_cdiv(t128, 256) * 256);
  if (cols == BIG_BN || deep_only) {
    if (dcols && (p.K + 63) / 64 <= DEEP_MAX_KT && (sw.deep == 2 || deep_only || (e256 < 0.40 && e128 < 0.40)))
      return set(Form::Deep, 128, dcols, dcols == 256 ? 3 : 4);
    if (deep_only) return;
  }
  if (e256 >= e128 && e256 >= 0.40) return set(Form::Tile, 256, cols, 2);
  if (e128 >= 0.40) return set(Form::Tile, 128, cols, 2);
  if (cols != BIG_BN) return;
  const SplitPlan sp128 = splitk_plan(p, vec4);
  if (sp128.splits && workspace_holds(p, sp128.splits)) return set(Form::SplitK, 128, BIG_BN, 2, sp128);
}

bool ln_fold_ok(const i2v_gemm_params& p, const GemmBigPlan& plan) {
  if (plan.form != GemmBigForm::Tile) return false;
  if (p.a_mode != I2V_A_PLAIN || p.a2 != nullptr) return false;
  if (p.rowvec && p.rowvec_period > 0 && (p.rowvec_period & (p.rowvec_period - 1)) != 0) return false;
  if (p.residual) return false;
  if (p.store_mode == I2V_STORE_ROWMAJOR || p.store_mode == I2V_STORE_ROWPERM)
    return p.epilogue == I2V_EPI_NONE || (p.epilogue == I2V_EPI_GEGLU && !p.rowvec);
  if (p.store_mode == I2V_STORE_VT_T)
    return p.vt_len % 8 == 0 && p.M % 8 == 0 && p.vt_ld % 8 == 0 && a16(p.c) &&
           (!p.rowvec || (p.rowvec_period >= 8 && (p.rowvec_period & (p.rowvec_period - 1)) == 0 && p.ld_rowvec % 8 == 0));
  return false;
}

int gn_partial_rows(const i2v_gemm_params& p, const GemmBigPlan& plan) {
  if (plan.form != GemmBigForm::Tile || plan.cols != BIG_BN) return 0;
  if (p.a_mode != I2V_A_CONV3X3 || p.epilogue != I2V_EPI_NONE || p.store_mode != I2V_STORE_ROWMAJOR) return 0;
  if (p.residual || p.ln_wsum || p.c_is_f32 || p.rows_per_w > 0 || p.a_perm_frames > 0) return 0;
  if (p.out_scale != 1.0f) return 0;
  if (p.gn_groups <= 0 || p.N % p.gn_groups != 0) return 0;
  const int cpg = p.N / p.gn_groups, hw = p.out_h * p.out_w;
  if (cpg <= 0 || BIG_BN % cpg != 0 || p.M % plan.rows != 0 || hw % plan.rows != 0) return 0;
  if (p.rowvec && (p.rowvec_period > 0 || p.rows_per_vec <= 0 || p.rows_per_vec % plan.rows != 0)) return 0;
  return plan.rows;
}

bool want_persistent(const i2v_gemm_params& p, const GemmBigPlan& plan) {
  const int mode = switches().persist;
  if (plan.form != GemmBigForm::Tile || plan.cols != BIG_BN || p.a_mode != I2V_A_PLAIN) return false;
  if (p.a2 != nullptr || p.M % plan.rows != 0 || lo_stream(p)) return false;
  return mode == 1 || (mode == 2 && p.ln_wsum != nullptr && p.epilogue == I2V_EPI_NONE && p.store_mode == I2V_STORE_ROWMAJOR);
}
int persistent_grid(int ntiles) {
  static const int cus = [] {
    int dev = 0, n = 0;
    if (hipGetDevice(&dev) != hipSuccess || hipDeviceGetAttribute(&n, hipDeviceAttributeMultiprocessorCount, dev) != hipSuccess)
      return 0;
    return n;
  }();
  return (cus > 0 && ntiles > cus) ? cus : ntiles;
}

bool want_4wave(const i2v_gemm_params& p, const GemmBigPlan& plan) {
#ifdef I2V_VARIANTS
  return switches().four_wave == 1 && plan.form == GemmBigForm::Tile && plan.cols == BIG_BN && p.a_mode == I2V_A_PLAIN &&
         p.K % 32 == 0 && !lo_stream(p);
#else
  return false;
#endif
}

enum BigExtra { EXTRA_NONE = 0, EXTRA_LNF = 1, EXTRA_HILO = 2, EXTRA_GNS = 4, EXTRA_UPF = 8 };

template <int BN, int NS, int AMODE, bool SPLIT, bool FAST, int NW>
constexpr bool big_kernel_exists(int epi, int store, int extra) {
  constexpr bool plain_a = AMODE == I2V_A_PLAIN;
  constexpr bool tile320 = BN == BIG_BN && NS == 2 && !SPLIT;
  constexpr bool deep = NS > 2;
  const bool rowmajor = store == I2V_STORE_ROWMAJOR, rowperm = store == I2V_STORE_ROWPERM;
  if (epi == I2V_EPI_GEGLU) return tile320 && plain_a && rowmajor && (extra == EXTRA_NONE || extra == EXTRA_LNF);
  if (epi != I2V_EPI_NONE) return false;
  switch (extra) {
    case EXTRA_NONE: return rowmajor || (plain_a && (tile320 || (deep && store != I2V_STORE_VT_T)));
    case EXTRA_LNF:  return tile320 && plain_a && store != I2V_STORE_VT;
    case EXTRA_HILO: return (tile320 || deep) && !FAST && NW == 8 && (rowmajor || (rowperm && plain_a));
    case EXTRA_GNS:  return tile320 && !plain_a && !FAST && NW == 8 && rowmajor;
    case EXTRA_UPF:  return NS == 2 && !SPLIT && !plain_a && !FAST && NW == 8 && rowmajor;
    default: return false;
  }
}

template <int... Vs, class F>
bool with_constant(int v, F&& f) {
  return ((v == Vs ? (f(std::integral_constant<int, Vs>{}), true) : false) || ...);
}

template <int BM, int BN, int NS, int AMODE, bool SPLIT = false, bool FAST = false, int NW = 8>
int launch_form(const i2v_gemm_params& p, const GemmBigPlan& plan, hipStream_t s, const char* what) {
  constexpr int BK = NW == 8 ? 64 : 32;
  const int tiles_n = p.N / BN, ntiles = (int)i2v_cdiv(p.M, BM) * tiles_n;
  const dim3 grid(FAST ? persistent_grid(ntiles) : ntiles, SPLIT ? plan.splits : 1), block(NW * 64);
  const int extra = (p.ln_wsum ? EXTRA_LNF : 0) | (lo_stream(p) && !SPLIT ? EXTRA_HILO : 0) | (p.gn_partial ? EXTRA_GNS : 0) |
                    (upconv_fold(p) ? EXTRA_UPF : 0);
  bool launched = false;
  with_constant<I2V_EPI_NONE, I2V_EPI_GEGLU>(p.epilogue, [&](auto epi) {
    with_constant<I2V_STORE_ROWMAJOR, I2V_STORE_ROWPERM, I2V_STORE_VT, I2V_STORE_VT_T>(p.store_mode, [&](auto store) {
      with_constant<EXTRA_NONE, EXTRA_LNF, EXTRA_HILO, EXTRA_GNS, EXTRA_UPF>(extra, [&](auto ex) {
        constexpr int EPI = decltype(epi)::value, STORE = decltype(store)::value, EX = decltype(ex)::value;
        if constexpr (big_kernel_exists<BN, NS, AMODE, SPLIT, FAST, NW>(EPI, STORE, EX)) {
          hipLaunchKernelGGL((gemm_big_kernel<BM, BK, NS, AMODE, EPI, STORE, SPLIT, NW == 8, EX == EXTRA_LNF, FAST, BN, NW,
                                              EX == EXTRA_GNS, EX == EXTRA_HILO, EX == EXTRA_UPF>),
                             grid, block, 0, s, p, tiles_n, plan.kps, ntiles);
          launched = true;
        }
      });
    });
  });
  if (!launched)
    I2V_FAIL(I2V_ERR_UNSUPPORTED, "%s: no kernel for epilogue %d, store %d, ln_wsum %d, hi + lo %d, gn_partial %d, folded up-sampling %d",
             what, p.epilogue, p.store_mode, p.ln_wsum != nullptr, (int)lo_stream(p), p.gn_partial != nullptr, (int)upconv_fold(p));
  const int rc = i2v_check_launch(what);
  return rc < 0 ? rc : 1;
}

template <int BN, int NS, int AMODE, bool SPLIT = false, bool FAST = false>
int launch_rows(const i2v_gemm_params& p, const GemmBigPlan& plan, hipStream_t s, const char* what) {
  return plan.rows == 256 ? launch_form<256, BN, NS, AMODE, SPLIT, FAST>(p, plan, s, what)
                          : launch_form<128, BN, NS, AMODE, SPLIT, FAST>(p, plan, s, what);
}

}

GemmBigPlan i2v_gemm_big_plan(const i2v_gemm_params& p, int vec4) {
  GemmBigPlan plan;
  if (switches().splitk != 0) {
    const int splits = std::max(splitk_plan(p, vec4).splits, splitk256_plan(p, vec4).splits);
    plan.workspace_bytes = (int64_t)splits * p.M * p.N * (int64_t)sizeof(float);
  }
  plan_form(p, vec4, plan);
  plan.four_wave = want_4wave(p, plan);
  plan.persistent = !plan.four_wave && want_persistent(p, plan);
  plan.ln_fold = ln_fold_ok(p, plan);
  plan.gn_rows = gn_partial_rows(p, plan);
  return plan;
}

#ifdef I2V_VARIANTS
int i2v_gemm_alt_try(const i2v_gemm_params& p, hipStream_t s);
#endif

int i2v_gemm_big_launch(const i2v_gemm_params& p, int vec4, const GemmBigPlan& plan, hipStream_t s) {
  constexpr int PLAIN = I2V_A_PLAIN, CONV = I2V_A_CONV3X3;
  const bool conv = p.a_mode == I2V_A_CONV3X3;
  switch (plan.form) {
    case GemmBigForm::None:
      return 0;
    case GemmBigForm::Tile:
      if (plan.cols == 256) return launch_rows<256, 2, CONV>(p, plan, s, "i2v_gemm_f16(big conv)");
      if (plan.cols == 128) return launch_rows<128, 2, CONV>(p, plan, s, "i2v_gemm_f16(big conv)");
#ifdef I2V_VARIANTS
      if (const int rc = i2v_gemm_alt_try(p, s); rc != 0) return rc;
      if (plan.four_wave) return launch_form<128, BIG_BN, 2, PLAIN, false, false, 4>(p, plan, s, "i2v_gemm_f16(big, 4-wave)");
#endif
      if (conv) return launch_rows<BIG_BN, 2, CONV>(p, plan, s, "i2v_gemm_f16(big)");
      if (plan.persistent && persistent_grid(1 << 20) != (1 << 20))
        return launch_rows<BIG_BN, 2, PLAIN, false, true>(p, plan, s, "i2v_gemm_f16(big, persistent)");
      return launch_rows<BIG_BN, 2, PLAIN>(p, plan, s, "i2v_gemm_f16(big)");
    case GemmBigForm::Deep:
      return plan.cols == 256 ? launch_form<128, 256, 3, PLAIN>(p, plan, s, "i2v_gemm_f16(big, deep pipeline)")
                              : launch_form<128, 128, 4, PLAIN>(p, plan, s, "i2v_gemm_f16(big, deep pipeline)");
    case GemmBigForm::SplitK: {
      const int rc = conv ? launch_rows<BIG_BN, 2, CONV, true>(p, plan, s, "i2v_gemm_f16(split-K)")
                          : launch_rows<BIG_BN, 2, PLAIN, true>(p, plan, s, "i2v_gemm_f16(split-K)");
      if (rc < 0) return rc;
      const int64_t groups = (int64_t)p.M * (p.N / 4);
      const int blocks = (int)(i2v_cdiv(groups, 256) < 2048 ? i2v_cdiv(groups, 256) : 2048);
      hipLaunchKernelGGL(splitk_reduce_kernel, dim3(blocks), dim3(256), 0, s, p, plan.splits, vec4);
      const int rc2 = i2v_check_launch("i2v_gemm_f16(split-K reduce)");
      return rc2 < 0 ? rc2 : 1;
    }
  }
  return 0;
}
```

i2v-adapter-unofficial_amd/csrc/gemm_common.h:

```cpp
#pragma once
#include "common.h"

__device__ __forceinline__ int gemm_swz(int row, int chunk) { return row * 128 + ((chunk ^ ((row >> 1) & 7)) << 4); }

struct GemmRow {
  int m;
  int64_t m_out;
  const f16* rv;
  const f16* rs;
  const f16* rl;
  f16* cl;
};

__device__ __forceinline__ f16 lo_half(const float v, const f16 hi) { return (f16)(v - (float)hi); }

__device__ __forceinline__ GemmRow gemm_make_row(const i2v_gemm_params& p, int m) {
  GemmRow r;
  r.m = m;
  r.m_out = m;
  if (p.store_mode == I2V_STORE_ROWPERM) {
    const int per = p.hw * p.frames;
    const int b = m / per, rem = m - b * per;
    const int pix = rem / p.frames, f = rem - pix * p.frames;
    r.m_out = (int64_t)(b * p.frames + f) * p.hw + pix;
  }
  const f16* rowvec = reinterpret_cast<const f16*>(p.rowvec);
  const f16* resid = reinterpret_cast<const f16*>(p.residual);
  r.rv = rowvec ? rowvec + (int64_t)(p.rowvec_period > 0 ? (m & (p.rowvec_period - 1)) : m / p.rows_per_vec) * p.ld_rowvec
                : nullptr;
  r.rs = resid ? resid + r.m_out * p.ldr : nullptr;
  r.rl = (resid && p.residual_lo) ? reinterpret_cast<const f16*>(p.residual_lo) + r.m_out * p.ldr : nullptr;
  r.cl = p.c_lo ? reinterpret_cast<f16*>(p.c_lo) + r.m_out * p.ldc : nullptr;
  return r;
}

__device__ __forceinline__ void gemm_store4(const i2v_gemm_params& p, const int vec4, const GemmRow& row, const int n,
                                            float v[4]) {
  const int N = p.N;
  if (n >= N) return;
  const f16* __restrict__ bias = reinterpret_cast<const f16*>(p.bias);
  f16* __restrict__ C = reinterpret_cast<f16*>(p.c);
  const float oscale = p.out_scale;
  if (vec4) {
    if (bias) {
      const f16x4 b4 = *reinterpret_cast<const f16x4*>(bias + n);
#pragma unroll
      for (int r = 0; r < 4; ++r) v[r] += (float)b4[r];
    }
    if (row.rv) {
      const f16x4 t4 = *reinterpret_cast<const f16x4*>(row.rv + n);
#pragma unroll
      for (int r = 0; r < 4; ++r) v[r] += (float)t4[r];
    }
    if (row.rs) {
      const f16x4 r4 = *reinterpret_cast<const f16x4*>(row.rs + n);
#pragma unroll
      for (int r = 0; r < 4; ++r) v[r] += (float)r4[r];
      if (row.rl) {
        const f16x4 l4 = *reinterpret_cast<const f16x4*>(row.rl + n);
#pragma unroll
        for (int r = 0; r < 4; ++r) v[r] += (float)l4[r];
      }
    }
  } else {
#pragma unroll
    for (int r = 0; r < 4; ++r) {
      if (n + r < N) {
        if (bias) v[r] += (float)bias[n + r];
        if (row.rv) v[r] += (float)row.rv[n + r];
        if (row.rs) v[r] += (float)row.rs[n + r];
        if (row.rl) v[r] += (float)row.rl[n + r];
      }
    }
  }
  if (p.epilogue == I2V_EPI_GEGLU) {
    const float o0 = v[0] * gelu_erf(v[1]) * oscale;
    const float o1 = v[2] * gelu_erf(v[3]) * oscale;
    f16* dst = C + row.m_out * p.ldc + (n >> 1);
    if (vec4) {
      f16x2 o = {(f16)o0, (f16)o1};
      *reinterpret_cast<f16x2*>(dst) = o;
    } else {
      if (n + 1 < N) dst[0] = (f16)o0;
      if (n + 3 < N) dst[1] = (f16)o1;
    }
    return;
  }
#pragma unroll
  for (int r = 0; r < 4; ++r) {
    if (p.epilogue == I2V_EPI_GELU) v[r] = gelu_erf(v[r]);
    v[r] *= oscale;
  }
  if (p.store_mode == I2V_STORE_VT) {
    if (vec4) {
      const int bt = n / p.vt_len, kk = n - bt * p.vt_len;
      f16x4 o = {(f16)v[0], (f16)v[1], (f16)v[2], (f16)v[3]};
      *reinterpret_cast<f16x4*>(C + ((int64_t)bt * p.M + row.m) * p.vt_ld + kk) = o;
    } else {
#pragma unroll
      for (int r = 0; r < 4; ++r) {
        if (n + r < N) {
          const int bt = (n + r) / p.vt_len, kk = (n + r) - bt * p.vt_len;
          C[((int64_t)bt * p.M + row.m) * p.vt_ld + kk] = (f16)v[r];
        }
      }
    }
  } else {
    f16* dst = C + row.m_out * p.ldc + n;
    if (vec4) {
      f16x4 o = {(f16)v[0], (f16)v[1], (f16)v[2], (f16)v[3]};
      *reinterpret_cast<f16x4*>(dst) = o;
      if (row.cl) *reinterpret_cast<f16x4*>(row.cl + n) = f16x4{lo_half(v[0], o[0]), lo_half(v[1], o[1]), lo_half(v[2], o[2]), lo_half(v[3], o[3])};
    } else {
#pragma unroll
      for (int r = 0; r < 4; ++r)
        if (n + r < N) {
          dst[r] = (f16)v[r];
          if (row.cl) row.cl[n + r] = lo_half(v[r], (f16)v[r]);
        }
    }
  }
}

enum class GemmBigForm { None, Tile, SplitK, Deep };
struct GemmBigPlan {
  GemmBigForm form = GemmBigForm::None;
  int rows = 0, cols = 0, stages = 0;
  int splits = 0, kps = 0;
  int64_t workspace_bytes = 0;
  bool persistent = false;
  bool four_wave = false;
  bool ln_fold = false;
  int gn_rows = 0;
};
GemmBigPlan i2v_gemm_big_plan(const i2v_gemm_params& p, int vec4);
int i2v_gemm_big_launch(const i2v_gemm_params& p, int vec4, const GemmBigPlan& plan, hipStream_t s);
int i2v_conv_thin_try(const i2v_gemm_params& p, hipStream_t s);
int i2v_gemm_ws_try(const i2v_gemm_params& p, hipStream_t s);
int i2v_gemm_ws_ok(const i2v_gemm_params& p);
```

i2v-adapter-unofficial_amd/kernels.py:

```python
import ctypes as C
import functools
import os
from typing import Optional

import torch

from . import _lib
from ._lib import (I2V_A_CONV3X3, I2V_A_PLAIN, I2V_EPI_GEGLU, I2V_EPI_GELU, I2V_EPI_NONE, I2V_STORE_ROWMAJOR,
                   I2V_STORE_ROWPERM, I2V_STORE_VT, I2V_STORE_VT_T, AttnBwdParams, AttnParams, GemmParams, GnParams,
                   HipLibraryError, LnParams, TAttnParams)

f16 = torch.float16


def _stream():
    return C.c_void_p(torch.cuda.current_stream().cuda_stream)


def _req(t: torch.Tensor, name: str, dtype=f16):
    if not isinstance(t, torch.Tensor):
        raise TypeError(f"{name} must be a tensor")
    if not t.is_cuda:
        raise HipLibraryError(f"{name} is on {t.device}: the I2V-Adapter HIP path has no CPU fallback "
                              "(move tensors to a ROCm device)")
# ... 24 lines not shown
    return None if t is None else getattr(t, "_i2v_lo", None)


def sview(t, *shape):
    v, lo = t.view(*shape), lo_of(t)
    if lo is not None:
        v._i2v_lo = lo.view(*shape)
    return v


def _attach_lo(p_res_lo_setter, residual, out):
    rl = lo_of(residual)
    if rl is not None and (rl.shape != residual.shape or rl.stride() != residual.stride() or rl.dtype != f16):
        raise ValueError("the low half of a stream tensor must be laid out like the tensor")
    cl = torch.empty_like(out)
    if cl.stride() != out.stride():
        raise ValueError("precise stream: `out` must be dense")
    p_res_lo_setter(rl, cl)
    out._i2v_lo = cl
    return rl, cl


def gemm(a, w, bias=None, *, a2=None, residual=None, rowvec=None, rows_per_vec=0, epilogue=I2V_EPI_NONE,
         out=None, store=I2V_STORE_ROWMAJOR, frames=0, hw=0, vt_len=0, vt_ld=0, out_scale=1.0, ln=None,
         rowvec_period=0, query_ln_support=False, w_rows=0, a_perm=None, query_batch_support=False, precise=False):
    lib = _lib.load()
    a, lda = _mat(a, "a")
    w_stack = None
    if w.dim() == 3:
        _req(w, "w")
        if w_rows <= 0 or not w.is_contiguous() or a.shape[0] != w.shape[0] * w_rows:
            raise ValueError(f"stacked w {tuple(w.shape)} needs contiguous storage and w_rows with S * w_rows == M")
        w_stack, w = w, w[0]
    w, ldw = _mat(w, "w")
    M, K1 = a.shape
    N, K = w.shape
    p = GemmParams()
    if w_stack is not None:
        p.w_batch_stride, p.rows_per_w = w_stack.stride(0), w_rows
    if a_perm is not None:
        p.a_perm_frames, p.a_perm_hw = int(a_perm[0]), int(a_perm[1])
    p.a, p.lda = _p(a), lda
    if a2 is not None:
        a2, lda2 = _mat(a2, "a2")
        if a2.shape[0] != M or K1 + a2.shape[1] != K:
            raise ValueError(f"dual-source A shapes {tuple(a.shape)} + {tuple(a2.shape)} do not match W {tuple(w.shape)}")
        p.a2, p.lda2, p.k_split = _p(a2), lda2, K1
    elif K1 != K:
        raise ValueError(f"A is {tuple(a.shape)} but W is {tuple(w.shape)}")
    p.a_mode = I2V_A_PLAIN
    p.w, p.ldw = _p(w), ldw
    if bias is not None:
        _req(bias, "bias")
        if bias.numel() != N or not bias.is_contiguous():
            raise ValueError("bias must be a contiguous vector of N elements")
        p.bias = _p(bias)
    n_out = N // 2 if epilogue == I2V_EPI_GEGLU else N
    if store in (I2V_STORE_VT, I2V_STORE_VT_T):
        tokens, chans = (N, M) if store == I2V_STORE_VT else (M, N)
        if out is None or vt_len <= 0 or vt_ld < vt_len or tokens % vt_len != 0:
            raise ValueError("VT store needs an `out` buffer, vt_len > 0, vt_ld >= vt_len and tokens % vt_len == 0")
        _req(out, "out")
        if not out.is_contiguous() or out.numel() < (tokens // vt_len) * chans * vt_ld:
            raise ValueError("VT `out` must be contiguous with at least (tokens / vt_len) * channels * vt_ld elements")
        p.c, p.ldc = _p(out), vt_ld
        p.vt_len, p.vt_ld = vt_len, vt_ld
    else:
        if out is None:
            out = torch.empty((M, n_out), dtype=f16, device=a.device)
        out, ldc = _mat(out, "out")
        if out.shape != (M, n_out):
            raise ValueError(f"out must be {(M, n_out)}, got {tuple(out.shape)}")
        p.c, p.ldc = _p(out), ldc
    if residual is not None:
        residual, ldr = _mat(residual, "residual")
        if residual.shape != (M, n_out) or epilogue == I2V_EPI_GEGLU:
            raise ValueError(f"residual must be {(M, n_out)} (and is not supported with GEGLU)")
        p.residual, p.ldr = _p(residual), ldr
    if rowvec is not None:
        rowvec, ldv = _mat(rowvec, "rowvec")
        if rowvec_period > 0:
            want = (N, rowvec_period) if store == I2V_STORE_VT_T else (rowvec_period, N)
            if rowvec.shape[0] < want[0] or rowvec.shape[1] < want[1] or (store != I2V_STORE_VT_T and rowvec.shape[1] != N):
                raise ValueError(f"periodic rowvec must cover {want}, got {tuple(rowvec.shape)}")
            p.rowvec, p.ld_rowvec, p.rowvec_period = _p(rowvec), ldv, rowvec_period
        else:
            if rows_per_vec <= 0 or M % rows_per_vec != 0 or rowvec.shape != (M // rows_per_vec, N):
                raise ValueError(f"rowvec must be [M / rows_per_vec, N], got {tuple(rowvec.shape)}")
            p.rowvec, p.ld_rowvec, p.rows_per_vec = _p(rowvec), ldv, rows_per_vec
    if ln is not None:
        wsum, eps = ln
        _req(wsum, "ln wsum", dtype=torch.float32)
        if wsum.numel() != N or not wsum.is_contiguous() or a2 is not None:
            raise ValueError(f"ln = (wsum fp32 [N], eps) with a single-source A expected, got {tuple(wsum.shape)}")
        p.ln_wsum, p.ln_eps = _p(wsum), float(eps)
    p.M, p.N, p.K = M, N, K
    p.epilogue, p.store_mode = epilogue, store
    p.frames, p.hw = frames, hw
    p.out_scale = out_scale
    if query_ln_support:
        return bool(lib.i2v_gemm_ln_supported(C.byref(p)))
    if query_batch_support:
        return bool(lib.i2v_gemm_batch_supported(C.byref(p)))
    keep = None
    if precise:
        if epilogue != I2V_EPI_NONE or store not in (I2V_STORE_ROWMAJOR, I2V_STORE_ROWPERM) or ln is not None:
            raise ValueError("precise=True needs a plain row-major / row-permuted store")

        def set_lo(rl, cl):
            p.residual_lo, p.c_lo = _p(rl), _p(cl)
        keep = _attach_lo(set_lo, residual, out)
    ws = _attach_splitk_workspace(lib, p, a.device)
    _lib.check(lib.i2v_gemm_f16(C.byref(p), _stream()), "i2v_gemm_f16")
    del ws, keep
    return out


def _attach_splitk_workspace(lib, p, device):
    need = lib.i2v_gemm_workspace_bytes(C.byref(p))
    if need <= 0:
        return None
    ws = torch.empty((need + 3) // 4, dtype=torch.float32, device=device)
    p.workspace, p.workspace_bytes = _p(ws), need
    return ws


def conv_k_block(cin: int) -> int:
    return 64 if cin % 64 == 0 and os.environ.get("I2V_CONV_KBLOCK", "1") != "0" else 0


def _upconv_fold_params(p, n, h, wd, cin, cout):
    p.a_mode, p.lda = I2V_A_CONV3X3, cin
    p.M, p.N, p.K, p.ldw, p.ldc = 4 * n * h * wd, cout, 4 * cin, 4 * cin, cout
    p.epilogue, p.store_mode, p.out_scale = I2V_EPI_NONE, I2V_STORE_ROWMAJOR, 1.0
    p.n_img, p.in_h, p.in_w, p.cin = n, h, wd, cin
    p.out_h, p.out_w, p.stride, p.upsample = 2 * h, 2 * wd, 1, 2
    p.conv_kblock = conv_k_block(cin)
    p.w_batch_stride, p.rows_per_w = cout * 4 * cin, n * h * wd


@functools.lru_cache(maxsize=None)
def _upconv_fold_query(n, h, wd, cin, cout, kblock):
    p = GemmParams()
    _upconv_fold_params(p, n, h, wd, cin, cout)
    p.a = p.w = p.c = p.bias = 1 << 40
    return bool(_lib.load().i2v_gemm_upconv_fold_supported(C.byref(p)))


def upconv_fold_supported(x_shape, cout):
    n, h, wd, cin = (int(v) for v in x_shape)
    return _upconv_fold_query(n, h, wd, cin, int(cout), conv_k_block(cin))


def conv3x3(x, w_packed, bias=None, *, stride=1, upsample=False, rowvec=None, rows_per_vec=0, residual=None,
            out_scale=1.0, asym_pad=False, out_f32=False, gn_stats_groups=0, precise=False, output_size=None, w_folded=None):
    lib = _lib.load()
    _req(x, "x")
    if x.dim() != 4 or not x.is_contiguous():
        raise ValueError(f"x must be a contiguous [N, H, W, C] tensor, got {tuple(x.shape)}")
    n, h, wd, cin = x.shape
    if w_folded is not None:
        if (not upsample or stride != 1 or asym_pad or rowvec is not None or residual is not None or out_scale != 1.0 or out_f32
                or gn_stats_groups or precise):
            raise ValueError("w_folded belongs to a plain up-sampling convolution (bias only)")
        if output_size is not None and tuple(int(v) for v in output_size) != (2 * h, 2 * wd):
            raise ValueError(f"w_folded: the folded form up-samples to exactly {(2 * h, 2 * wd)}, not {tuple(output_size)}")
        _req(w_folded, "w_folded")
        cout = w_folded.shape[1] if w_folded.dim() == 3 else 0
        if tuple(w_folded.shape) != (4, cout, 4 * cin) or not w_folded.is_contiguous():
            raise ValueError(f"w_folded must be a contiguous [4, Cout, {4 * cin}] tensor, got {tuple(w_folded.shape)}")
        out = torch.empty((n, 2 * h, 2 * wd, cout), dtype=f16, device=x.device)
        p = GemmParams()
        _upconv_fold_params(p, n, h, wd, cin, cout)
        p.a, p.w, p.c = _p(x), _p(w_folded), _p(out)
        if bias is not None:
            _req(bias, "bias")
            if bias.numel() != cout or not bias.is_contiguous():
                raise ValueError("bias must be a contiguous vector of Cout elements")
            p.bias = _p(bias)
        _lib.check(lib.i2v_gemm_f16(C.byref(p), _stream()), "i2v_gemm_f16(conv3x3, folded up-sampling)")
        return out
    w_packed, ldw = _mat(w_packed, "w_packed")
    cout, K = w_packed.shape
    if K != 9 * cin:
        raise ValueError(f"w_packed is {tuple(w_packed.shape)} but x has {cin} channels")
    if asym_pad and (stride != 2 or upsample):
        raise ValueError("asym_pad needs stride 2 and no upsampling")
    if upsample:
        if stride != 1:
            raise ValueError("upsample conv must have stride 1")
        oh, ow = 2 * h, 2 * wd
        if output_size is not None:
            oh, ow = int(output_size[0]), int(output_size[1])
            if oh not in (2 * h, 2 * h - 1) or ow not in (2 * wd, 2 * wd - 1):
                raise NotImplementedError(f"upsample to {(oh, ow)} from {(h, wd)}: only 2x and 2x - 1 (a level that was odd before its "
                                          "stride-2 down-sampler) occur on the UNet's path")
    else:
        if output_size is not None:
            raise ValueError("output_size belongs to an upsampling convolution")
        padsum = 1 if asym_pad else 2
        oh, ow = (h + padsum - 3) // stride + 1, (wd + padsum - 3) // stride + 1
    M = n * oh * ow
    if out_f32 and (cout > 64 or residual is not None):
        raise ValueError("out_f32 is for narrow outputs (Cout <= 64) without a residual")
    out = torch.empty((n, oh, ow, cout), dtype=torch.float32 if out_f32 else f16, device=x.device)
    p = GemmParams()
    p.c_is_f32 = 1 if out_f32 else 0
    p.a, p.lda = _p(x), cin
    p.a_mode = I2V_A_CONV3X3
    p.w, p.ldw = _p(w_packed), ldw
    if bias is not None:
        _req(bias, "bias")
        if bias.numel() != cout or not bias.is_contiguous():
            raise ValueError("bias must be a contiguous vector of Cout elements")
        p.bias = _p(bias)
    if residual is not None:
        _req(residual, "residual")
        if tuple(residual.shape) != (n, oh, ow, cout) or not residual.is_contiguous():
            raise ValueError(f"residual must be contiguous {(n, oh, ow, cout)}")
        p.residual, p.ldr = _p(residual), cout
    if rowvec is not None:
        rowvec, ldv = _mat(rowvec, "rowvec")
        if rows_per_vec <= 0 or M % rows_per_vec != 0 or rowvec.shape != (M // rows_per_vec, cout):
            raise ValueError(f"rowvec must be [M / rows_per_vec, Cout], got {tuple(rowvec.shape)}")
        p.rowvec, p.ld_rowvec, p.rows_per_vec = _p(rowvec), ldv, rows_per_vec
    p.c, p.ldc = _p(out), cout
    p.M, p.N, p.K = M, cout, K
    p.epilogue, p.store_mode = I2V_EPI_NONE, I2V_STORE_ROWMAJOR
    p.out_scale = out_scale
    p.n_img, p.in_h, p.in_w, p.cin = n, h, wd, cin
    p.out_h, p.out_w, p.stride, p.upsample = oh, ow, stride, 1 if upsample else 0
    p.asym_pad = 1 if asym_pad else 0
    p.conv_kblock = conv_k_block(cin)
    keep = None
    if precise:
        if out_f32 or gn_stats_groups:
            raise ValueError("precise=True is an fp16 result without GroupNorm partials")

        def set_lo(rl, cl):
            p.residual_lo, p.c_lo = _p(rl), _p(cl)
        keep = _attach_lo(set_lo, residual, out)
    ws = _attach_splitk_workspace(lib, p, x.device)
    stats = None
    if gn_stats_groups:
        p.gn_groups = int(gn_stats_groups)
        rows = lib.i2v_gemm_gn_partial_rows(C.byref(p))
        if rows > 0:
            part = torch.empty((n, (oh * ow) // rows, int(gn_stats_groups), 2), dtype=torch.float32, device=x.device)
            p.gn_partial = _p(part)
            stats = (part, rows)
    _lib.check(lib.i2v_gemm_f16(C.byref(p), _stream()), "i2v_gemm_f16(conv3x3)")
    del ws, keep
    return (out, stats) if gn_stats_groups else out


def project_vt(tokens, w_v, batch_len, out=None, bias=None, ln=None, pe_t=None, pe_period=0, query_ln_support=False):
    tokens, _ = _mat(tokens, "tokens")
    T = tokens.shape[0]
    if T % batch_len != 0:
        raise ValueError(f"{T} tokens are not a multiple of batch_len {batch_len}")
    ld = pad8(batch_len)
    Cc = w_v.shape[0]
    natural = Cc % 320 == 0 and batch_len % 4 == 0 and T >= 8192
    if out is None:
        out = torch.empty((T // batch_len, Cc, ld), dtype=f16, device=tokens.device)
    if query_ln_support:
        return natural and gemm(tokens, w_v, bias, store=I2V_STORE_VT_T, vt_len=batch_len, vt_ld=ld, ln=ln, rowvec=pe_t,
                                rowvec_period=pe_period, out=out, query_ln_support=True)
    if natural:
        gemm(tokens, w_v, bias, store=I2V_STORE_VT_T, vt_len=batch_len, vt_ld=ld, out=out, ln=ln, rowvec=pe_t,
             rowvec_period=pe_period)
    else:
        if ln is not None or pe_t is not None or bias is not None:
            raise ValueError("the LayerNorm-folded V^T projection needs the natural operand order "
                             "(C % 320 == 0, batch_len % 4 == 0, >= 8192 tokens)")
        gemm(w_v, tokens, store=I2V_STORE_VT, vt_len=batch_len, vt_ld=ld, out=out)
    return out



def attention(q, k, vt, *, batch_q, lq, lk, heads, head_dim, kv_group=1, scale=None, out=None, accumulate=False,
              acc_scale=1.0, return_lse=False):
    lib = _lib.load()
    q, ldq = _mat(q, "q")
    k, ldk = _mat(k, "k")
    _req(vt, "vt")
    Cc = heads * head_dim
    bkv = batch_q // kv_group
    if q.shape[0] != batch_q * lq or q.shape[1] < Cc:
        raise ValueError(f"q is {tuple(q.shape)}, expected [{batch_q * lq}, >={Cc}]")
    if k.shape[0] != bkv * lk or k.shape[1] < Cc:
        raise ValueError(f"k is {tuple(k.shape)}, expected [{bkv * lk}, >={Cc}]")
    if vt.dim() != 3 or not vt.is_contiguous() or vt.shape[0] != bkv or vt.shape[1] != Cc or vt.shape[2] < pad8(lk):
        raise ValueError(f"vt is {tuple(vt.shape)}, expected contiguous [{bkv}, {Cc}, >={pad8(lk)}]")
    if out is None:
        if accumulate:
            raise ValueError("accumulate needs the `out` tensor holding the previous result")
        out = torch.empty((batch_q * lq, Cc), dtype=f16, device=q.device)
    out, ldo = _mat(out, "out")
    if out.shape[0] != batch_q * lq or out.shape[1] < Cc:
        raise ValueError("bad `out` shape")
    p = AttnParams()
    p.q, p.q_row_stride, p.q_batch_stride = _p(q), ldq, lq * ldq
    p.k, p.k_row_stride, p.k_batch_stride = _p(k), ldk, lk * ldk
    p.vt, p.vt_row_stride, p.vt_batch_stride = _p(vt), vt.shape[2], Cc * vt.shape[2]
    p.o, p.o_row_stride, p.o_batch_stride = _p(out), ldo, lq * ldo
    p.batch_q, p.kv_group, p.heads, p.head_dim, p.lq, p.lk = batch_q, kv_group, heads, head_dim, lq, lk
    p.scale = float(head_dim) ** -0.5 if scale is None else scale
    p.accumulate, p.acc_scale = 1 if accumulate else 0, acc_scale
    lse = None
    if return_lse:
        if accumulate:
            raise ValueError("return_lse is not combined with accumulate")
        if return_lse == "fused":
            lse = torch.empty((batch_q, heads, lq), dtype=torch.float32, device=q.device)
            p.lse = _p(lse)
        elif return_lse is not True:
            raise ValueError(f"return_lse must be False, True or 'fused', got {return_lse!r}")
    _lib.check(lib.i2v_attention_f16(C.byref(p), _stream()), "i2v_attention_f16")
    if return_lse and lse is None:
        lse = attention_lse(q, k, batch_q=batch_q, lq=lq, lk=lk, heads=heads, head_dim=head_dim, kv_group=kv_group, scale=p.scale)
    return (out, lse) if return_lse else out


def temporal_attention(q, k, vt, *, n_pixels, frames, heads, head_dim, scale=None):
    lib = _lib.load()
    q, ldq = _mat(q, "q")
    k, ldk = _mat(k, "k")
    _req(vt, "vt")
    Cc = heads * head_dim
    if q.shape[0] != n_pixels * frames or k.shape[0] != n_pixels * frames or q.shape[1] < Cc or k.shape[1] < Cc:
        raise ValueError("q / k must be [n_pixels * frames, >= C]")
    if vt.dim() != 3 or not vt.is_contiguous() or vt.shape[0] != n_pixels or vt.shape[1] != Cc or \
            vt.shape[2] < pad8(frames):
        raise ValueError(f"vt is {tuple(vt.shape)}, expected contiguous [{n_pixels}, {Cc}, >={pad8(frames)}]")
    out = torch.empty((n_pixels * frames, Cc), dtype=f16, device=q.device)
    p = TAttnParams()
    p.q, p.q_row_stride = _p(q), ldq
    p.k, p.k_row_stride = _p(k), ldk
    p.vt, p.vt_ld = _p(vt), vt.shape[2]
    p.o, p.o_row_stride = _p(out), Cc
    p.n_pixels, p.frames, p.heads, p.head_dim = n_pixels, frames, heads, head_dim
    p.scale = float(head_dim) ** -0.5 if scale is None else scale
    _lib.check(lib.i2v_temporal_attention_f16(C.byref(p), _stream()), "i2v_temporal_attention_f16")
    return out


def motion_attn_supported(rows, channels, heads, head_dim, frames):
    return bool(_lib.load().i2v_motion_attn_supported(rows, channels, heads, head_dim, frames))


def _pack_head_fragments(weights, heads):
    c_out, c_in = weights[0].shape
    d = c_out // heads
    dp = (d + 15) // 16 * 16
    n = len(weights)
    w = torch.zeros((heads, n, dp, c_in), dtype=f16, device=weights[0].device)
    for i, t in enumerate(weights):
        w[:, i, :d] = t.detach().to(f16).view(heads, d, c_in)
    w = w.view(heads, n, dp // 16, 16, c_in // 32, 4, 8).permute(0, 1, 4, 2, 5, 3, 6)
    return w.contiguous().view(heads * n * dp, c_in)


def pack_motion_qkv(wq, wk, wv, heads):
    w = _pack_head_fragments((wq, wk, wv), heads)
    if w.shape[0] != _lib.load().i2v_motion_attn_pack_rows(heads, wq.shape[0] // heads):
        raise RuntimeError("pack_motion_qkv: row count differs from i2v_motion_attn_pack_rows")
    return w


def pack_cross_q(wq, heads):
    w = _pack_head_fragments((wq,), heads)
    if w.shape[0] != _lib.load().i2v_cross_attn_fused_pack_rows(heads, wq.shape[0] // heads):
        raise RuntimeError("pack_cross_q: row count differs from i2v_cross_attn_fused_pack_rows")
    return w


def cross_attn_fused_supported(rows, channels, heads, head_dim, ctx_len, rows_per_ctx):
    return bool(_lib.load().i2v_cross_attn_fused_supported(rows, channels, heads, head_dim, ctx_len, rows_per_ctx))


def pack_ctx_fragments(k, vt, heads, ctx_len, out=None):
    lib = _lib.load()
    k, ldk = _mat(k, "k")
    _req(vt, "vt")
    if vt.dim() != 3 or vt.stride(2) != 1:
# ... 899 lines not shown
```

i2v-adapter-unofficial_amd/profiling.py:

```python
import torch

from . import kernels as K


def _numel_bytes(*ts):
    return sum(t.numel() * t.element_size() for t in ts if isinstance(t, torch.Tensor))


def _work_gemm(args, kw, out):
    a, w = args[0], args[1]
    M, N, Kd = a.shape[0], w.shape[-2], w.shape[-1]
    tag = "".join(t for t, on in ((" geglu", kw.get("epilogue") == K.I2V_EPI_GEGLU), (" gelu", kw.get("epilogue") == K.I2V_EPI_GELU),
                                  (" +res", kw.get("residual") is not None), (" +ln", kw.get("ln") is not None),
                                  (" st%d" % kw.get("store", 0), bool(kw.get("store")))) if on)
    if w.dim() == 3:
        tag += " wstack%d" % w.shape[0] + (" perm" if kw.get("a_perm") is not None else "")
    return ("gemm", 2.0 * M * N * Kd, _numel_bytes(a, kw.get("a2"), w, kw.get("residual"), out),
            f"{M}x{N}x{Kd}{tag}")


def _work_conv(args, kw, out):
    x, w = args[0], args[1]
    stats = None
    if isinstance(out, tuple):
        out, stats = out
    M = out.shape[0] * out.shape[1] * out.shape[2]
    wf = kw.get("w_folded")
    if wf is not None:
        return ("conv3x3", 2.0 * M * wf.shape[1] * wf.shape[2], _numel_bytes(x, wf, out), f"{M}x{wf.shape[1]}x{wf.shape[2]} up4")
    return ("conv3x3", 2.0 * M * w.shape[0] * w.shape[1], _numel_bytes(x, w, kw.get("residual"), out),
            f"{M}x{w.shape[0]}x{w.shape[1]}" + (" s2" if kw.get("stride", 1) == 2 else "")
            + (" up" if kw.get("upsample") else "") + (" +res" if kw.get("residual") is not None else "")
            + (" +gn stats" if stats is not None else ""))


def _work_attn(args, kw, out):
    c = kw["heads"] * kw["head_dim"]
    return ("attention", 4.0 * kw["batch_q"] * kw["lq"] * kw["lk"] * c, _numel_bytes(args[0], args[1], args[2], out),
            f"B{kw['batch_q']} Lq{kw['lq']} Lk{kw['lk']} h{kw['heads']} d{kw['head_dim']}")


def _work_tattn(args, kw, out):
    c = kw["heads"] * kw["head_dim"]
    return ("temporal_attention", 4.0 * kw["n_pixels"] * kw["frames"] * kw["frames"] * c,
            _numel_bytes(args[0], args[1], out) + kw["n_pixels"] * c * kw["frames"] * 2,
            f"px{kw['n_pixels']} F{kw['frames']} h{kw['heads']} d{kw['head_dim']}")


def _work_mattn(args, kw, out):
    x, w = args[0], args[3]
    rows, c = x.shape
    op = kw.get("out_proj")
    return ("motion_attn", 2.0 * rows * c * (4 if op else 3) * c + 4.0 * rows * kw["frames"] * c,
            _numel_bytes(x, w, out) + (_numel_bytes(x, op[0]) if op else 0),
            f"{rows}x{c} F{kw['frames']} h{kw['heads']} d{kw['head_dim']} (LN + q,k,v + attention" + (" + to_out + residual)" if op else ")"))


def _work_cattn(args, kw, out):
    x, w = args[0], args[3]
    rows, c = x.shape
    op = kw.get("out_proj")
    return ("cross_attn_fused", 2.0 * rows * c * (2 if op else 1) * c + 4.0 * rows * kw["ctx_len"] * c,
            _numel_bytes(x, w, args[4], out) + (_numel_bytes(x, op[0]) if op else 0),
            f"{rows}x{c} Lk{kw['ctx_len']} h{kw['heads']} d{kw['head_dim']} (LN + q + text attention" + (" + to_out + residual)" if op else ")"))


def _work_ff(args, kw, out):
    x = args[0]
    rows, c = x.shape
    inner = args[3][1].numel() // 2
    tail = kw.get("tail")
    if tail is not None:
        return ("ff_fused", 2.0 * rows * c * 2 * inner + 2.0 * rows * inner * c + 2.0 * rows * c * c,
                _numel_bytes(x, args[3][0], args[3][2], tail[0][0], tail[1], out),
                f"{rows}x{c} inner {inner} (LN + GEGLU FF + residual + proj_out + residual{', rows permuted' if tail[2] else ''})")
    return ("ff_fused", 2.0 * rows * c * 2 * inner + 2.0 * rows * inner * c, _numel_bytes(x, args[3][0], args[3][2], out),
            f"{rows}x{c} inner {inner} (LN + GEGLU FF + residual)")


def _work_lnqkv(args, kw, out):
    x, w = args[0], args[3]
    rows, c = x.shape
    return ("ln_qkv", 2.0 * rows * c * (kw["n_qk"] + c), _numel_bytes(x, w, out[0], out[1]),
            f"{rows}x{kw['n_qk']}+{c}x{c} (LN + q,k[,q_adapter] + V^T)")


def _work_gn(args, kw, out):
    if kw.get("stats") is not None:
        return "groupnorm", 0.0, 2 * _numel_bytes(out), "x".join(map(str, out.shape)) + " (stats given)"
    return "groupnorm", 0.0, 3 * _numel_bytes(out), "x".join(map(str, out.shape))


def _work_gn_fold(args, kw, out):
    x = args[0]
    return "groupnorm", 0.0, _numel_bytes(x, kw.get("x2")), "fold " + "x".join(map(str, x.shape))


def _work_ln(args, kw, out):
    return "layernorm", 0.0, 2 * _numel_bytes(out), "x".join(map(str, out.shape))


def _work_misc(name):
    def f(args, kw, out):
        return name, 0.0, 2 * _numel_bytes(out), ""
    return f


_WRAPPED = {
    "gemm": _work_gemm, "conv3x3": _work_conv, "attention": _work_attn, "temporal_attention": _work_tattn,
    "motion_attn": _work_mattn, "cross_attn_fused": _work_cattn, "ff_fused": _work_ff, "ln_qkv": _work_lnqkv,
    "groupnorm": _work_gn, "groupnorm_fold": _work_gn_fold, "layernorm": _work_ln, "silu": _work_misc("elementwise"),
    "copy3d": _work_misc("elementwise"), "timestep_embedding": _work_misc("elementwise"),
    "ddim_prep": _work_misc("elementwise"), "ddim_cfg_step": _work_misc("elementwise"),
    "nchw_to_tokens": _work_misc("elementwise"), "tokens_to_nchw": _work_misc("elementwise"),
}


class KernelProfile:
    def __init__(self):
        self.records = []
        self._saved = {}
        self._depth = 0

    def _wrap(self, name, fn, work):
        def wrapped(*args, **kw):
            if self._depth or kw.get("query_ln_support"):
                return fn(*args, **kw)
            s, e = torch.cuda.Event(enable_timing=True), torch.cuda.Event(enable_timing=True)
            self._depth += 1
            s.record()
            try:
                out = fn(*args, **kw)
            finally:
                self._depth -= 1
            e.record()
            cls, flops, nbytes, detail = work(args, kw, out)
            self.records.append((cls, flops, nbytes, s, e, f"{name} {detail}".strip()))
            return out
        return wrapped

    def __enter__(self):
        for name, work in _WRAPPED.items():
            self._saved[name] = getattr(K, name)
            setattr(K, name, self._wrap(name, self._saved[name], work))
        return self

    def __exit__(self, *exc):
        for name, fn in self._saved.items():
            setattr(K, name, fn)
        self._saved = {}

    def summary(self):
        return self._aggregate(lambda rec: rec[0])

    def by_shape(self):
        return self._aggregate(lambda rec: rec[5])

    def _aggregate(self, key):
        torch.cuda.synchronize()
        agg = {}
        for rec in self.records:
            cls, flops, nbytes, s, e = rec[:5]
            d = agg.setdefault(key(rec), dict(calls=0, ms=0.0, flops=0.0, bytes=0.0))
            d["calls"] += 1
            d["ms"] += s.elapsed_time(e)
            d["flops"] += flops
            d["bytes"] += nbytes
        for d in agg.values():
            sec = max(d["ms"], 1e-9) * 1e-3
            d["tflops"] = d["flops"] / sec / 1e12
            d["gbps"] = d["bytes"] / sec / 1e9
        return agg
```

include/i2v_hip.h:

```cpp
#ifndef I2V_HIP_H
#define I2V_HIP_H

#include <stdint.h>

#ifdef __cplusplus
extern "C" {
#endif

#define I2V_ABI_VERSION 11

#define I2V_OK 0
#define I2V_ERR_INVALID_ARG (-1)
#define I2V_ERR_UNSUPPORTED (-2)
#define I2V_ERR_LAUNCH (-3)

typedef void* i2v_stream_t;

int i2v_abi_version(void);
const char* i2v_last_error(void);

enum {
  I2V_EPI_NONE = 0,
  I2V_EPI_GELU = 1,
  I2V_EPI_GEGLU = 2
};

enum {
  I2V_STORE_ROWMAJOR = 0,
  I2V_STORE_ROWPERM = 1,
  I2V_STORE_VT = 2,
  I2V_STORE_VT_T = 3
};

enum {
  I2V_A_PLAIN = 0,
  I2V_A_CONV3X3 = 1
};

typedef struct i2v_gemm_params {
  const void* a;
  int64_t lda;
  const void* a2;
  int64_t lda2;
  int32_t k_split;
  int32_t a_mode;
  const void* w;
  int64_t ldw;
  const void* bias;
  const void* residual;
  int64_t ldr;
  const void* rowvec;
  int64_t ld_rowvec;
  int32_t rows_per_vec;
  int32_t rowvec_period;
  const void* ln_wsum;
  float ln_eps;
  void* c;
  int64_t ldc;
  int32_t M, N, K;
  int32_t epilogue;
  int32_t store_mode;
  int32_t frames, hw;
  int32_t vt_len, vt_ld;
  float out_scale;
  int32_t n_img, in_h, in_w, cin, out_h, out_w, stride, upsample, asym_pad;
  int32_t conv_kblock;
  int64_t w_batch_stride;
  int32_t rows_per_w;
  int32_t a_perm_frames, a_perm_hw;
  void* workspace;
  int64_t workspace_bytes;
  int32_t c_is_f32;
  void* gn_partial;
  int32_t gn_groups;
  const void* residual_lo;
  void* c_lo;
} i2v_gemm_params;

int i2v_gemm_f16(const i2v_gemm_params* p, i2v_stream_t stream);
int i2v_gemm_ln_supported(const i2v_gemm_params* p);
int i2v_gemm_batch_supported(const i2v_gemm_params* p);
int i2v_gemm_upconv_fold_supported(const i2v_gemm_params* p);
int64_t i2v_gemm_workspace_bytes(const i2v_gemm_params* p);
int32_t i2v_gemm_gn_partial_rows(const i2v_gemm_params* p);

typedef struct i2v_attn_params {
  const void* q;  int64_t q_row_stride, q_batch_stride;
  const void* k;  int64_t k_row_stride, k_batch_stride;
  const void* vt; int64_t vt_row_stride, vt_batch_stride;
  void* o;        int64_t o_row_stride, o_batch_stride;
  int32_t batch_q, kv_group, heads, head_dim, lq, lk;
  float scale;
  int32_t accumulate;
  float acc_scale;
  float* lse;
} i2v_attn_params;

int i2v_attention_f16(const i2v_attn_params* p, i2v_stream_t stream);

typedef struct i2v_tattn_params {
  const void* q; int64_t q_row_stride;
  const void* k; int64_t k_row_stride;
  const void* vt; int32_t vt_ld;
  void* o; int64_t o_row_stride;
  int32_t n_pixels, frames, heads, head_dim;
  float scale;
} i2v_tattn_params;

int i2v_temporal_attention_f16(const i2v_tattn_params* p, i2v_stream_t stream);

typedef struct i2v_motion_attn_params {
  const void* x; int64_t ldx;
  const void* gamma;
  const void* shift; int64_t ld_shift;
  const void* w_qkv;
  void* out; int64_t ldo;
  int64_t rows;
  int32_t channels, heads, head_dim, frames;
  float eps, scale;
  const void* w_o; const void* b_o;
} i2v_motion_attn_params;

int32_t i2v_motion_attn_supported(int64_t rows, int32_t channels, int32_t heads, int32_t head_dim, int32_t frames);
int32_t i2v_motion_attn_pack_rows(int32_t heads, int32_t head_dim);
int i2v_motion_attn_f16(const i2v_motion_attn_params* p, i2v_stream_t stream);

typedef struct i2v_cross_attn_fused_params {
  const void* x; int64_t ldx;
  const void* gamma; const void* beta;
  const void* w_q;
  const void* ctx_frag;
  void* out; int64_t ldo;
  int64_t rows, rows_per_ctx;
  int32_t channels, heads, head_dim, ctx_len;
  float eps, scale;
  const void* ip_frag; int32_t ip_len; float ip_scale;
  const void* w_o; const void* b_o;
} i2v_cross_attn_fused_params;

int32_t i2v_cross_attn_fused_supported(int64_t rows, int32_t channels, int32_t heads, int32_t head_dim, int32_t ctx_len,
                                       int64_t rows_per_ctx);
int32_t i2v_cross_attn_fused_pack_rows(int32_t heads, int32_t head_dim);
int64_t i2v_cross_attn_fused_ctx_elems(int32_t n_ctx, int32_t heads, int32_t head_dim);
int i2v_cross_attn_fused_f16(const i2v_cross_attn_fused_params* p, i2v_stream_t stream);

typedef struct i2v_ln_qkv_params {
  const void* x; int64_t ldx;
  const void* gamma; const void* beta;
  const void* w;
  void* qk; int64_t ld_qk;
  void* vt; int64_t vt_batch_stride, vt_row_stride;
  int64_t rows, rows_per_image;
  int32_t channels, n_qk;
  float eps;
  int64_t x_image_stride;
} i2v_ln_qkv_params;

int32_t i2v_ln_qkv_supported(int64_t rows, int32_t channels, int32_t n_qk, int64_t rows_per_image);
int i2v_ln_qkv_f16(const i2v_ln_qkv_params* p, i2v_stream_t stream);

typedef struct i2v_ff_fused_params {
  const void* x; int64_t ldx;
  const void* gamma; const void* beta;
  const void* w1; const void* b1;
  const void* w2; const void* b2;
  void* out; int64_t ldo;
  int64_t rows;
  int32_t channels, inner;
  float eps;
  const void* w3; const void* b3;
  const void* res2; int64_t ld_res2;
  int32_t perm_frames, perm_hw;
  const void* res2_lo;
  void* out_lo;
} i2v_ff_fused_params;

int32_t i2v_ff_fused_supported(int64_t rows, int32_t channels, int32_t inner);
int32_t i2v_ff_fused_tail_supported(int64_t rows, int32_t channels, int32_t inner, int32_t perm_frames, int32_t perm_hw);
int i2v_ff_fused_f16(const i2v_ff_fused_params* p, i2v_stream_t stream);

typedef struct i2v_gn_params {
  const void* x;  int32_t c1;
  const void* x2; int32_t c2;
  const void* gamma; const void* beta;
  void* y;
  int32_t n_img, hw, groups, frames_per_stat;
  float eps;
  int32_t silu;
  int32_t out_perm; int32_t frames;
  void* workspace;
  const void* gpartial_in; int32_t gpartial_rows;
} i2v_gn_params;

int64_t i2v_groupnorm_workspace_bytes(int32_t n_img, int32_t hw, int32_t channels);
int i2v_groupnorm_f16(const i2v_gn_params* p, i2v_stream_t stream);
int i2v_groupnorm_fold_f16(const i2v_gn_params* p, const void* w, int64_t ldw, const void* bias, int32_t n_out,
                           void* w_out, void* bias_out, i2v_stream_t stream);

typedef struct i2v_ln_params {
  const void* x; int64_t ldx;
  const void* gamma; const void* beta;
  const void* pe; int64_t ld_pe; int32_t pe_period;
  void* y; int64_t ldy;
  int32_t rows, C;
  float eps;
  int32_t x_rows_per_batch; int64_t x_batch_stride;
} i2v_ln_params;

int i2v_layernorm_f16(const i2v_ln_params* p, i2v_stream_t stream);

int i2v_softmax_rows_f16(const void* x, int64_t ldx, void* y, int64_t ldy, int32_t rows, int32_t cols, float scale,
                         i2v_stream_t stream);

int i2v_nchw_to_tokens(const void* src, int32_t src_is_f32, void* dst, int32_t n, int32_t c, int32_t hw,
                       int32_t c_pad, i2v_stream_t stream);
int i2v_tokens_to_nchw(const void* src, int32_t src_is_f32, int64_t ld, void* dst, int32_t dst_is_f32, int32_t n,
                       int32_t c, int32_t hw, i2v_stream_t stream);
int i2v_timestep_embedding(const float* t, const int32_t* t_index, int32_t t_rows, void* out, int32_t n,
                           int32_t dim, i2v_stream_t stream);
int i2v_select_row_f16(const void* table, int64_t ld, int32_t rows, const int32_t* row_index, void* out, int32_t cols,
                       i2v_stream_t stream);
int i2v_silu_f16(const void* x, void* y, int64_t n, i2v_stream_t stream);
int i2v_repeat_rows_f16(const void* x, void* y, int64_t rows_in, int64_t cols, int32_t repeat,
                        i2v_stream_t stream);
int i2v_copy3d_f16(const void* src, int64_t src_batch_stride, int64_t ld_src, void* dst, int64_t dst_batch_stride,
                   int64_t ld_dst, int64_t batches, int64_t rows, int64_t cols, i2v_stream_t stream);

int64_t i2v_pack_ctx_fragments_elems(int32_t n_ctx, int32_t heads, int32_t head_dim);
int i2v_pack_ctx_fragments_f16(const void* k, int64_t ldk, const void* vt, int64_t vt_row_stride, int64_t vt_batch_stride, void* out,
                               int32_t n_ctx, int32_t heads, int32_t head_dim, int32_t ctx_len, i2v_stream_t stream);

int i2v_ddim_prep(float* latents, const float* cond, void* model_in, int32_t b, int32_t f, int32_t c,
                  int32_t hw, int32_t c_pad, int32_t cfg_copies, i2v_stream_t stream);
int i2v_ddim_cfg_step(float* latents, const void* noise_pred, int32_t np_is_f32, int64_t ld_np, const float* coef, int32_t n_steps,
                      int32_t* step_index, float guidance_scale, int32_t b, int32_t f, int32_t c, int32_t hw,
// ... 120 lines not shown
```

Before: 21.32.

## Fold ResNet 1x1 shortcut GEMM into conv2 as a K-dimension tail

For ResNet blocks with a 1x1 conv_shortcut, the shortcut weights are concatenated onto the packed conv2 weights along K, and the conv kernel gains a TAIL mode. In that mode the extra K blocks are loaded straight from the block input (and the optional concat input), so one GEMM produces conv2 plus shortcut with the two biases pre-summed. This removes the separate shortcut GEMM, the side-stream fork, and the residual read and write. It adds a new kernel instantiation and restricts the fold to stride-1, 320-column, non-precise convolutions, and the longer K may change the split or tile choice.

```diff
diff --git a/i2v-adapter-unofficial_amd/_lib.py b/i2v-adapter-unofficial_amd/_lib.py
--- a/i2v-adapter-unofficial_amd/_lib.py
+++ b/i2v-adapter-unofficial_amd/_lib.py
@@ -3,7 +3,7 @@
 
 _HERE = os.path.dirname(os.path.abspath(__file__))
 LIB_PATH = os.environ.get("I2V_LIB_PATH") or os.path.join(_HERE, "libi2v_hip.so")
-ABI_VERSION = 11
+ABI_VERSION = 12
 
 I2V_EPI_NONE, I2V_EPI_GELU, I2V_EPI_GEGLU = 0, 1, 2
 I2V_STORE_ROWMAJOR, I2V_STORE_ROWPERM, I2V_STORE_VT, I2V_STORE_VT_T = 0, 1, 2, 3
@@ -39,6 +39,8 @@
         ("c_is_f32", C.c_int32),
         ("gn_partial", C.c_void_p), ("gn_groups", C.c_int32),
         ("residual_lo", C.c_void_p), ("c_lo", C.c_void_p),
+        ("tail_a", C.c_void_p), ("ld_tail", C.c_int64), ("tail_a2", C.c_void_p), ("ld_tail2", C.c_int64),
+        ("tail_k", C.c_int32), ("tail_split", C.c_int32),
     ]
 
 
@@ -197,6 +199,7 @@
     "i2v_gemm_ln_supported": (C.c_int, [C.POINTER(GemmParams)]),
     "i2v_gemm_batch_supported": (C.c_int, [C.POINTER(GemmParams)]),
     "i2v_gemm_upconv_fold_supported": (C.c_int, [C.POINTER(GemmParams)]),
+    "i2v_gemm_conv_tail_supported": (C.c_int, [C.POINTER(GemmParams)]),
     "i2v_gemm_workspace_bytes": (C.c_int64, [C.POINTER(GemmParams)]),
     "i2v_gemm_gn_partial_rows": (C.c_int32, [C.POINTER(GemmParams)]),
     "i2v_attention_f16": (C.c_int, [C.POINTER(AttnParams), _P]),
diff --git a/i2v-adapter-unofficial_amd/blocks.py b/i2v-adapter-unofficial_amd/blocks.py
--- a/i2v-adapter-unofficial_amd/blocks.py
+++ b/i2v-adapter-unofficial_amd/blocks.py
@@ -90,6 +90,18 @@
     if K.conv_k_block(ci):
         w = w.reshape(co, 9, ci // 64, 64).permute(0, 2, 1, 3)
     return w.reshape(co, 9 * ci).to(f16).contiguous()
+
+
+def pack_conv3x3_tail(w2: torch.Tensor, ws: torch.Tensor, dtype=f16) -> torch.Tensor:
+    co = w2.shape[0]
+    w = w2.detach().permute(0, 2, 3, 1)
+    c = w.shape[3]
+    if K.conv_k_block(c):
+        w = w.reshape(co, 9, c // 64, 64).permute(0, 2, 1, 3)
+    return torch.cat([w.reshape(co, 9 * c), ws.detach().reshape(co, -1)], dim=1).to(dtype).contiguous()
+
+
+SHORTCUT_FOLD = os.environ.get("I2V_SHORTCUT_FOLD", "1") != "0"
 
 
 def pack_upconv_fold(weight: torch.Tensor, dtype=f16) -> torch.Tensor:
@@ -297,14 +309,16 @@
                               if in_channels != out_channels else None)
 
     def _pack(self):
-        p = dict(g1=w16(self.norm1.weight), b1=w16(self.norm1.bias), w1=pack_conv3x3(self.conv1.weight),
-                 cb1=w16(self.conv1.bias), g2=w16(self.norm2.weight), b2=w16(self.norm2.bias),
-                 w2=pack_conv3x3(self.conv2.weight), cb2=w16(self.conv2.bias))
+        p = LazyPack(g1=w16(self.norm1.weight), b1=w16(self.norm1.bias), w1=pack_conv3x3(self.conv1.weight),
+                     cb1=w16(self.conv1.bias), g2=w16(self.norm2.weight), b2=w16(self.norm2.bias),
+                     w2=pack_conv3x3(self.conv2.weight), cb2=w16(self.conv2.bias))
         if self.time_emb_proj is not None:
             p["wt"], p["bt"] = w16(self.time_emb_proj.weight), w16(self.time_emb_proj.bias)
         if self.conv_shortcut is not None:
             p["ws"] = w16(self.conv_shortcut.weight.reshape(self.out_channels, self.in_channels))
             p["bs"] = w16(self.conv_shortcut.bias)
+            p.lazy("w2s", lambda: pack_conv3x3_tail(self.conv2.weight, self.conv_shortcut.weight))
+            p.lazy("cb2s", lambda: (self.conv2.bias.detach().float() + self.conv_shortcut.bias.detach().float()).to(f16).contiguous())
         return p
 
     def _fwd(self, x, temb_act, x2=None):
@@ -316,8 +330,10 @@
         if self.conv_shortcut is None and x2 is not None:
             raise ValueError("concat input needs a conv_shortcut")
         s = x
-        with streams.fork(self.conv_shortcut is not None and n * hh * ww <= streams.MAX_ROWS, x.device) as fk:
-            if self.conv_shortcut is not None:
+        fold = (SHORTCUT_FOLD and self.conv_shortcut is not None and not precise_stream()
+                and K.conv_tail_supported((n, hh, ww, self.out_channels), self.out_channels, c1, cin - c1))
+        with streams.fork(self.conv_shortcut is not None and not fold and n * hh * ww <= streams.MAX_ROWS, x.device) as fk:
+            if self.conv_shortcut is not None and not fold:
                 with fk.side():
                     a2 = None if x2 is None else x2.view(-1, x2.shape[3])
                     s = K.sview(K.gemm(x.view(-1, c1), p["ws"], p["bs"], a2=a2, precise=precise_stream()), n, hh, ww, self.out_channels)
@@ -332,6 +348,9 @@
             else:
                 h, st = K.conv3x3(h, p["w1"], p["cb1"], rowvec=rowvec, rows_per_vec=rpv), None
             h = K.groupnorm(h, p["g2"], p["b2"], self.groups, self.eps, silu=True, stats=st)
+        if fold:
+            return K.conv3x3(h, p["w2s"], p["cb2s"], out_scale=1.0 / self.output_scale_factor,
+                             tail=(x.view(-1, c1), None if x2 is None else x2.view(-1, x2.shape[3])))
         return K.conv3x3(h, p["w2"], p["cb2"], residual=s, out_scale=1.0 / self.output_scale_factor, precise=precise_stream())
 
     def forward(self, input_tensor, temb, scale: float = 1.0):
diff --git a/i2v-adapter-unofficial_amd/csrc/gemm.hip b/i2v-adapter-unofficial_amd/csrc/gemm.hip
--- a/i2v-adapter-unofficial_amd/csrc/gemm.hip
+++ b/i2v-adapter-unofficial_amd/csrc/gemm.hip
@@ -361,6 +361,11 @@
   return i2v_gemm_big_plan(*pp, vector_epilogue_ok(*pp)).form == GemmBigForm::Tile ? 1 : 0;
 }
 
+extern "C" int i2v_gemm_conv_tail_supported(const i2v_gemm_params* pp) {
+  if (pp == nullptr || pp->M <= 0 || pp->N <= 0 || pp->K <= 0 || pp->a_mode != I2V_A_CONV3X3 || pp->tail_k <= 0) return 0;
+  return i2v_gemm_big_plan(*pp, vector_epilogue_ok(*pp)).tail ? 1 : 0;
+}
+
 extern "C" int32_t i2v_gemm_gn_partial_rows(const i2v_gemm_params* pp) {
   if (pp == nullptr) return 0;
   return i2v_gemm_big_plan(*pp, vector_epilogue_ok(*pp)).gn_rows;
@@ -380,8 +385,9 @@
   if (p.a_mode == I2V_A_CONV3X3) {
     I2V_CHECK_ARG(p.a2 == nullptr, "i2v_gemm_f16: conv mode takes a single source");
     I2V_CHECK_ARG(p.upsample >= 0 && p.upsample <= 2, "i2v_gemm_f16: upsample must be 0, 1 or 2 (got %d)", p.upsample);
-    I2V_CHECK_ARG(p.cin > 0 && p.cin % 8 == 0 && p.K == (p.upsample == 2 ? 4 : 9) * p.cin,
-                  "i2v_gemm_f16: conv needs cin %% 8 == 0, K == 9 cin (4 cin with the up-sampling folded into the weights)");
+    I2V_CHECK_ARG(p.tail_k >= 0 && (p.tail_k == 0 || p.upsample == 0), "i2v_gemm_f16: a K tail (tail_k %d) belongs to a convolution without up-sampling", p.tail_k);
+    I2V_CHECK_ARG(p.cin > 0 && p.cin % 8 == 0 && (int64_t)p.K == (p.upsample == 2 ? 4ll : 9ll) * p.cin + p.tail_k,
+                  "i2v_gemm_f16: conv needs cin %% 8 == 0, K == 9 cin (4 cin with the up-sampling folded into the weights; 9 cin + tail_k with a K tail)");
     I2V_CHECK_ARG(p.stride == 1 || p.stride == 2, "i2v_gemm_f16: conv stride must be 1 or 2");
     I2V_CHECK_ARG(!(p.upsample && p.stride != 1), "i2v_gemm_f16: upsample conv must have stride 1");
     I2V_CHECK_ARG(!p.asym_pad || (p.stride == 2 && !p.upsample), "i2v_gemm_f16: asym_pad needs stride 2, no upsample");
@@ -397,6 +403,7 @@
     I2V_CHECK_ARG((int64_t)p.n_img * p.in_h * p.in_w < (1ll << 31), "i2v_gemm_f16: conv image too large");
   } else {
     I2V_CHECK_ARG(p.a_mode == I2V_A_PLAIN, "i2v_gemm_f16: bad a_mode %d", p.a_mode);
+    I2V_CHECK_ARG(p.tail_k == 0, "i2v_gemm_f16: a K tail (tail_k) belongs to an I2V_A_CONV3X3 problem");
     if (p.a2) {
       I2V_CHECK_ARG(p.k_split > 0 && p.k_split < p.K && p.k_split % 8 == 0 && p.lda2 % 8 == 0 && aligned_to(p.a2, 16),
                     "i2v_gemm_f16: bad dual-source split (k_split %d, K %d)", p.k_split, p.K);
@@ -464,6 +471,11 @@
     I2V_FAIL(I2V_ERR_INVALID_ARG, "i2v_gemm_f16: the folded up-sampling convolution (upsample = 2) is not implemented for this problem "
              "(M %d N %d cin %d, %d x %d -> %d x %d, rows_per_w %d): ask i2v_gemm_upconv_fold_supported() first", p.M, p.N, p.cin,
              p.in_h, p.in_w, p.out_h, p.out_w, p.rows_per_w);
+  if (p.tail_k > 0 && !big_plan.tail)
+    I2V_FAIL(I2V_ERR_INVALID_ARG, "i2v_gemm_f16: the convolution with a plain-source K tail is not implemented for this problem "
+             "(M %d N %d cin %d tail %d split %d, stride %d, upsample %d, rowvec %d, ln_wsum %d, gn_partial %d, hi + lo %d): ask "
+             "i2v_gemm_conv_tail_supported() first", p.M, p.N, p.cin, p.tail_k, p.tail_a2 ? p.tail_split : 0, p.stride, p.upsample,
+             p.rowvec != nullptr, p.ln_wsum != nullptr, p.gn_partial != nullptr, (p.residual_lo || p.c_lo) ? 1 : 0);
   if (p.rows_per_w > 0 || p.a_perm_frames > 0) {
     I2V_CHECK_ARG(p.rows_per_w >= 0 && p.a_perm_frames >= 0 && p.w_batch_stride >= 0, "i2v_gemm_f16: negative batch / permutation field");
     if (big_plan.form != GemmBigForm::Tile)
diff --git a/i2v-adapter-unofficial_amd/csrc/gemm_big.hip b/i2v-adapter-unofficial_amd/csrc/gemm_big.hip
--- a/i2v-adapter-unofficial_amd/csrc/gemm_big.hip
+++ b/i2v-adapter-unofficial_amd/csrc/gemm_big.hip
@@ -57,7 +57,7 @@
 }
 
 template <int BM, int BK, int NS, int AMODE, int EPI, int STORE, bool SPLIT = false, bool STAGGER = true, bool LNF = false,
-          bool FAST = false, int BNT = 320, int NW = 8, bool GNS = false, bool HILO = false, bool UPF = false>
+          bool FAST = false, int BNT = 320, int NW = 8, bool GNS = false, bool HILO = false, bool UPF = false, bool TAIL = false>
 __global__ __launch_bounds__(NW * 64, NW == 4 ? 2 : 1) void gemm_big_kernel(const i2v_gemm_params p, const int tiles_n,
                                                                             const int kps, const int ntiles) {
   static_assert(NS == 2 || (NS <= 4 && !FAST && !SPLIT && NW == 8),
@@ -66,6 +66,9 @@
   static_assert(!UPF || (AMODE == I2V_A_CONV3X3 && EPI == I2V_EPI_NONE && STORE == I2V_STORE_ROWMAJOR && !SPLIT && !LNF && !FAST &&
                          !GNS && !HILO && NW == 8),
                 "the folded up-sampling convolution is an un-split conv with the plain row-contiguous store");
+  static_assert(!TAIL || (AMODE == I2V_A_CONV3X3 && EPI == I2V_EPI_NONE && STORE == I2V_STORE_ROWMAJOR && !LNF && !FAST && !GNS &&
+                          !HILO && !UPF && NW == 8 && BNT == 320 && BK == 64 && NS == 2),
+                "the plain-source K tail belongs to the 320-column convolution with the plain row-contiguous store");
   constexpr int BN = BNT;
   constexpr int WNC = BN / 4;
   constexpr int WM = BM / (NW / 4), MI = WM / 16, NI = WNC / 16;
@@ -112,6 +115,13 @@
   const auto rs_a = __builtin_amdgcn_make_buffer_rsrc(const_cast<f16*>(A), 0, (int)(a_extent * 2), 0x00020000);
   const auto rs_a2 = __builtin_amdgcn_make_buffer_rsrc(
       const_cast<f16*>(A2 ? A2 : A), 0, A2 ? (int)(((int64_t)(M - 1) * p.lda2 + (K - ksp)) * 2) : 0, 0x00020000);
+  const int kconv = TAIL ? K - p.tail_k : K;
+  const int tsp = (TAIL && p.tail_a2 != nullptr) ? p.tail_split : p.tail_k;
+  const auto rs_t = __builtin_amdgcn_make_buffer_rsrc(const_cast<void*>(TAIL ? p.tail_a : p.a), 0,
+                                                      TAIL ? (int)(((int64_t)(M - 1) * p.ld_tail + tsp) * 2) : 0, 0x00020000);
+  const auto rs_t2 = __builtin_amdgcn_make_buffer_rsrc(
+      const_cast<void*>((TAIL && p.tail_a2) ? p.tail_a2 : p.a), 0,
+      (TAIL && p.tail_a2) ? (int)(((int64_t)(M - 1) * p.ld_tail2 + (p.tail_k - tsp)) * 2) : 0, 0x00020000);
   const int pf = p.a_perm_frames;
   const int pf_shift = pf > 0 ? 31 - __builtin_clz(pf) : 0;
   const unsigned a_lane = pf > 0 ? (unsigned)((((r0 & (pf - 1)) * p.a_perm_hw + (r0 >> pf_shift)) * (int)p.lda + lane_k) * 2)
@@ -147,7 +157,19 @@
     char* sa = smem + stage * STAGE;
     char* sw = sa + BM * BK * 2;
     const int kb = kt * BK;
-    if (AMODE == I2V_A_CONV3X3) {
+    if (TAIL && kb >= kconv) {
+      const int tk = kb - kconv;
+      const bool first = tk < tsp;
+#pragma unroll
+      for (int i = 0; i < AG; ++i) {
+        const int m = tm0 + r0 + RSTEP * i;
+        const unsigned voff = m < M ? (unsigned)((m * (int)(first ? p.ld_tail : p.ld_tail2) + lane_k) * 2) : OOB;
+        if (first)
+          bdma16(rs_t, sa + (wave + NW * i) * 1024, voff, tk * 2);
+        else
+          bdma16(rs_t2, sa + (wave + NW * i) * 1024, voff, (tk - tsp) * 2);
+      }
+    } else if (AMODE == I2V_A_CONV3X3) {
       int tap, ci;
       if (UPF && p.conv_kblock) {
         tap = kt & 3;
@@ -866,6 +888,8 @@
 
 bool upconv_fold(const i2v_gemm_params& p) { return p.a_mode == I2V_A_CONV3X3 && p.upsample == 2; }
 
+bool conv_tail(const i2v_gemm_params& p) { return p.a_mode == I2V_A_CONV3X3 && p.tail_k > 0; }
+
 struct SplitPlan {
   int splits = 0, kps = 0;
 };
@@ -968,6 +992,17 @@
   if ((int64_t)p.M * p.ldc >= (1ll << 30) || (p.residual && (int64_t)p.M * p.ldr >= (1ll << 30)) ||
       (p.rowvec && rv_rows * p.ld_rowvec >= (1ll << 30)))
     return;
+  if (p.tail_k != 0) {
+    if (!conv || p.tail_k < 0 || cols != BIG_BN || p.stride != 1 || p.upsample != 0 || p.asym_pad) return;
+    if (p.rowvec || p.ln_wsum || p.gn_partial || lo_stream(p) || p.rows_per_w > 0 || p.a_perm_frames > 0) return;
+    if (p.tail_k % 64 != 0 || (int64_t)p.K != 9ll * p.cin + p.tail_k) return;
+    if (!p.tail_a || !a16(p.tail_a) || p.ld_tail % 8 != 0 || (int64_t)p.M * p.ld_tail >= (1ll << 30)) return;
+    const int tsp = p.tail_a2 ? p.tail_split : p.tail_k;
+    if (p.tail_a2 && (!a16(p.tail_a2) || p.ld_tail2 % 8 != 0 || tsp <= 0 || tsp >= p.tail_k || tsp % 64 != 0 ||
+                      p.ld_tail2 < p.tail_k - tsp || (int64_t)p.M * p.ld_tail2 >= (1ll << 30)))
+      return;
+    if (p.ld_tail < tsp) return;
+  }
   const bool fold = upconv_fold(p);
   if (fold) {
     if (p.K != 4 * p.cin || p.stride != 1 || p.out_h != 2 * p.in_h || p.out_w != 2 * p.in_w) return;
@@ -1007,6 +1042,7 @@
   if (cols != BIG_BN) return;
   const SplitPlan sp128 = splitk_plan(p, vec4);
   if (sp128.splits && workspace_holds(p, sp128.splits)) return set(Form::SplitK, 128, BIG_BN, 2, sp128);
+  if (conv_tail(p)) return set(Form::Tile, 128, BIG_BN, 2);
 }
 
 bool ln_fold_ok(const i2v_gemm_params& p, const GemmBigPlan& plan) {
@@ -1025,7 +1061,7 @@
 int gn_partial_rows(const i2v_gemm_params& p, const GemmBigPlan& plan) {
   if (plan.form != GemmBigForm::Tile || plan.cols != BIG_BN) return 0;
   if (p.a_mode != I2V_A_CONV3X3 || p.epilogue != I2V_EPI_NONE || p.store_mode != I2V_STORE_ROWMAJOR) return 0;
-  if (p.residual || p.ln_wsum || p.c_is_f32 || p.rows_per_w > 0 || p.a_perm_frames > 0) return 0;
+  if (p.residual || p.ln_wsum || p.c_is_f32 || p.rows_per_w > 0 || p.a_perm_frames > 0 || p.tail_k != 0) return 0;
   if (p.out_scale != 1.0f) return 0;
   if (p.gn_groups <= 0 || p.N % p.gn_groups != 0) return 0;
   const int cpg = p.N / p.gn_groups, hw = p.out_h * p.out_w;
@@ -1059,7 +1095,7 @@
 #endif
 }
 
-enum BigExtra { EXTRA_NONE = 0, EXTRA_LNF = 1, EXTRA_HILO = 2, EXTRA_GNS = 4, EXTRA_UPF = 8 };
+enum BigExtra { EXTRA_NONE = 0, EXTRA_LNF = 1, EXTRA_HILO = 2, EXTRA_GNS = 4, EXTRA_UPF = 8, EXTRA_TAIL = 16 };
 
 template <int BN, int NS, int AMODE, bool SPLIT, bool FAST, int NW>
 constexpr bool big_kernel_exists(int epi, int store, int extra) {
@@ -1075,6 +1111,7 @@
     case EXTRA_HILO: return (tile320 || deep) && !FAST && NW == 8 && (rowmajor || (rowperm && plain_a));
     case EXTRA_GNS:  return tile320 && !plain_a && !FAST && NW == 8 && rowmajor;
     case EXTRA_UPF:  return NS == 2 && !SPLIT && !plain_a && !FAST && NW == 8 && rowmajor;
+    case EXTRA_TAIL: return BN == BIG_BN && NS == 2 && !plain_a && !FAST && NW == 8 && rowmajor;
     default: return false;
   }
 }
@@ -1090,15 +1127,15 @@
   const int tiles_n = p.N / BN, ntiles = (int)i2v_cdiv(p.M, BM) * tiles_n;
   const dim3 grid(FAST ? persistent_grid(ntiles) : ntiles, SPLIT ? plan.splits : 1), block(NW * 64);
   const int extra = (p.ln_wsum ? EXTRA_LNF : 0) | (lo_stream(p) && !SPLIT ? EXTRA_HILO : 0) | (p.gn_partial ? EXTRA_GNS : 0) |
-                    (upconv_fold(p) ? EXTRA_UPF : 0);
+                    (upconv_fold(p) ? EXTRA_UPF : 0) | (conv_tail(p) ? EXTRA_TAIL : 0);
   bool launched = false;
   with_constant<I2V_EPI_NONE, I2V_EPI_GEGLU>(p.epilogue, [&](auto epi) {
     with_constant<I2V_STORE_ROWMAJOR, I2V_STORE_ROWPERM, I2V_STORE_VT, I2V_STORE_VT_T>(p.store_mode, [&](auto store) {
-      with_constant<EXTRA_NONE, EXTRA_LNF, EXTRA_HILO, EXTRA_GNS, EXTRA_UPF>(extra, [&](auto ex) {
+      with_constant<EXTRA_NONE, EXTRA_LNF, EXTRA_HILO, EXTRA_GNS, EXTRA_UPF, EXTRA_TAIL>(extra, [&](auto ex) {
         constexpr int EPI = decltype(epi)::value, STORE = decltype(store)::value, EX = decltype(ex)::value;
         if constexpr (big_kernel_exists<BN, NS, AMODE, SPLIT, FAST, NW>(EPI, STORE, EX)) {
           hipLaunchKernelGGL((gemm_big_kernel<BM, BK, NS, AMODE, EPI, STORE, SPLIT, NW == 8, EX == EXTRA_LNF, FAST, BN, NW,
-                                              EX == EXTRA_GNS, EX == EXTRA_HILO, EX == EXTRA_UPF>),
+                                              EX == EXTRA_GNS, EX == EXTRA_HILO, EX == EXTRA_UPF, EX == EXTRA_TAIL>),
                              grid, block, 0, s, p, tiles_n, plan.kps, ntiles);
           launched = true;
         }
@@ -1106,8 +1143,9 @@
     });
   });
   if (!launched)
-    I2V_FAIL(I2V_ERR_UNSUPPORTED, "%s: no kernel for epilogue %d, store %d, ln_wsum %d, hi + lo %d, gn_partial %d, folded up-sampling %d",
-             what, p.epilogue, p.store_mode, p.ln_wsum != nullptr, (int)lo_stream(p), p.gn_partial != nullptr, (int)upconv_fold(p));
+    I2V_FAIL(I2V_ERR_UNSUPPORTED, "%s: no kernel for epilogue %d, store %d, ln_wsum %d, hi + lo %d, gn_partial %d, folded up-sampling %d, K tail %d",
+             what, p.epilogue, p.store_mode, p.ln_wsum != nullptr, (int)lo_stream(p), p.gn_partial != nullptr, (int)upconv_fold(p),
+             (int)conv_tail(p));
   const int rc = i2v_check_launch(what);
   return rc < 0 ? rc : 1;
 }
@@ -1131,6 +1169,7 @@
   plan.persistent = !plan.four_wave && want_persistent(p, plan);
   plan.ln_fold = ln_fold_ok(p, plan);
   plan.gn_rows = gn_partial_rows(p, plan);
+  plan.tail = conv_tail(p) && (plan.form == GemmBigForm::Tile || plan.form == GemmBigForm::SplitK);
   return plan;
 }
 
diff --git a/i2v-adapter-unofficial_amd/csrc/gemm_common.h b/i2v-adapter-unofficial_amd/csrc/gemm_common.h
--- a/i2v-adapter-unofficial_amd/csrc/gemm_common.h
+++ b/i2v-adapter-unofficial_amd/csrc/gemm_common.h
@@ -132,6 +132,7 @@
   bool four_wave = false;
   bool ln_fold = false;
   int gn_rows = 0;
+  bool tail = false;
 };
 GemmBigPlan i2v_gemm_big_plan(const i2v_gemm_params& p, int vec4);
 int i2v_gemm_big_launch(const i2v_gemm_params& p, int vec4, const GemmBigPlan& plan, hipStream_t s);
diff --git a/i2v-adapter-unofficial_amd/kernels.py b/i2v-adapter-unofficial_amd/kernels.py
--- a/i2v-adapter-unofficial_amd/kernels.py
+++ b/i2v-adapter-unofficial_amd/kernels.py
@@ -200,8 +200,37 @@
     return _upconv_fold_query(n, h, wd, cin, int(cout), conv_k_block(cin))
 
 
+def _conv_tail_params(p, n, h, wd, cin, cout, k1, k2, ld1=None, ld2=None):
+    p.a_mode, p.lda = I2V_A_CONV3X3, cin
+    p.M, p.N, p.K = n * h * wd, cout, 9 * cin + k1 + k2
+    p.ldw, p.ldc = p.K, cout
+    p.epilogue, p.store_mode, p.out_scale = I2V_EPI_NONE, I2V_STORE_ROWMAJOR, 1.0
+    p.n_img, p.in_h, p.in_w, p.cin = n, h, wd, cin
+    p.out_h, p.out_w, p.stride, p.upsample = h, wd, 1, 0
+    p.conv_kblock = conv_k_block(cin)
+    p.tail_k, p.ld_tail = k1 + k2, k1 if ld1 is None else ld1
+    if k2:
+        p.tail_split, p.ld_tail2 = k1, k2 if ld2 is None else ld2
+
+
+@functools.lru_cache(maxsize=None)
+def _conv_tail_query(n, h, wd, cin, cout, k1, k2, kblock):
+    p = GemmParams()
+    _conv_tail_params(p, n, h, wd, cin, cout, k1, k2)
+    p.a = p.w = p.c = p.bias = p.tail_a = 1 << 40
+    if k2:
+        p.tail_a2 = 1 << 40
+    return bool(_lib.load().i2v_gemm_conv_tail_supported(C.byref(p)))
+
+
+def conv_tail_supported(x_shape, cout, k1, k2=0):
+    n, h, wd, cin = (int(v) for v in x_shape)
+    return _conv_tail_query(n, h, wd, cin, int(cout), int(k1), int(k2), conv_k_block(cin))
+
+
 def conv3x3(x, w_packed, bias=None, *, stride=1, upsample=False, rowvec=None, rows_per_vec=0, residual=None,
-            out_scale=1.0, asym_pad=False, out_f32=False, gn_stats_groups=0, precise=False, output_size=None, w_folded=None):
+            out_scale=1.0, asym_pad=False, out_f32=False, gn_stats_groups=0, precise=False, output_size=None, w_folded=None,
+            tail=None):
     lib = _lib.load()
     _req(x, "x")
     if x.dim() != 4 or not x.is_contiguous():
@@ -230,8 +259,22 @@
         return out
     w_packed, ldw = _mat(w_packed, "w_packed")
     cout, K = w_packed.shape
-    if K != 9 * cin:
-        raise ValueError(f"w_packed is {tuple(w_packed.shape)} but x has {cin} channels")
+    t1 = t2 = None
+    if tail is not None:
+        t1, t2 = tail
+        if stride != 1 or upsample or asym_pad or rowvec is not None or out_f32 or gn_stats_groups or precise:
+            raise ValueError("tail belongs to a plain stride-1 convolution (bias, residual and out_scale only)")
+        t1, ld_t1 = _mat(t1, "tail[0]")
+        ld_t2 = 0
+        if t2 is not None:
+            t2, ld_t2 = _mat(t2, "tail[1]")
+        k_tail = t1.shape[1] + (t2.shape[1] if t2 is not None else 0)
+        if t1.shape[0] != n * h * wd or (t2 is not None and t2.shape[0] != n * h * wd):
+            raise ValueError(f"tail sources must have one row per output pixel ({n * h * wd})")
+    else:
+        k_tail = 0
+    if K != 9 * cin + k_tail:
+        raise ValueError(f"w_packed is {tuple(w_packed.shape)} but x has {cin} channels" + (f" and the tail {k_tail} columns" if k_tail else ""))
     if asym_pad and (stride != 2 or upsample):
         raise ValueError("asym_pad needs stride 2 and no upsampling")
     if upsample:
@@ -280,6 +323,10 @@
     p.out_h, p.out_w, p.stride, p.upsample = oh, ow, stride, 1 if upsample else 0
     p.asym_pad = 1 if asym_pad else 0
     p.conv_kblock = conv_k_block(cin)
+    if t1 is not None:
+        p.tail_a, p.ld_tail, p.tail_k = _p(t1), ld_t1, k_tail
+        if t2 is not None:
+            p.tail_a2, p.ld_tail2, p.tail_split = _p(t2), ld_t2, t1.shape[1]
     keep = None
     if precise:
         if out_f32 or gn_stats_groups:
diff --git a/i2v-adapter-unofficial_amd/profiling.py b/i2v-adapter-unofficial_amd/profiling.py
--- a/i2v-adapter-unofficial_amd/profiling.py
+++ b/i2v-adapter-unofficial_amd/profiling.py
@@ -28,9 +28,10 @@
     wf = kw.get("w_folded")
     if wf is not None:
         return ("conv3x3", 2.0 * M * wf.shape[1] * wf.shape[2], _numel_bytes(x, wf, out), f"{M}x{wf.shape[1]}x{wf.shape[2]} up4")
-    return ("conv3x3", 2.0 * M * w.shape[0] * w.shape[1], _numel_bytes(x, w, kw.get("residual"), out),
+    return ("conv3x3", 2.0 * M * w.shape[0] * w.shape[1], _numel_bytes(x, w, kw.get("residual"), out, *(kw.get("tail") or ())),
             f"{M}x{w.shape[0]}x{w.shape[1]}" + (" s2" if kw.get("stride", 1) == 2 else "")
             + (" up" if kw.get("upsample") else "") + (" +res" if kw.get("residual") is not None else "")
+            + (" +tail%d" % (w.shape[1] - 9 * x.shape[3]) if kw.get("tail") is not None else "")
             + (" +gn stats" if stats is not None else ""))
 
 
diff --git a/include/i2v_hip.h b/include/i2v_hip.h
--- a/include/i2v_hip.h
+++ b/include/i2v_hip.h
@@ -7,7 +7,7 @@
 extern "C" {
 #endif
 
-#define I2V_ABI_VERSION 11
+#define I2V_ABI_VERSION 12
 
 #define I2V_OK 0
 #define I2V_ERR_INVALID_ARG (-1)
@@ -75,12 +75,18 @@
   int32_t gn_groups;
   const void* residual_lo;
   void* c_lo;
+  const void* tail_a;
+  int64_t ld_tail;
+  const void* tail_a2;
+  int64_t ld_tail2;
+  int32_t tail_k, tail_split;
 } i2v_gemm_params;
 
 int i2v_gemm_f16(const i2v_gemm_params* p, i2v_stream_t stream);
 int i2v_gemm_ln_supported(const i2v_gemm_params* p);
 int i2v_gemm_batch_supported(const i2v_gemm_params* p);
 int i2v_gemm_upconv_fold_supported(const i2v_gemm_params* p);
+int i2v_gemm_conv_tail_supported(const i2v_gemm_params* p);
 int64_t i2v_gemm_workspace_bytes(const i2v_gemm_params* p);
 int32_t i2v_gemm_gn_partial_rows(const i2v_gemm_params* p);
 
```

After: 21.41 (median of 6 runs). About the same (+0.4%).
